# Sovik-Ghosh/SFM

Hardware: AMD Instinct MI355X
Metric: BA LM-iterations/sec + descriptor-pairs/sec, 200 cams / 100k pts, 1->8 MI355X (higher is better)
Workload: dtype f64; 1 GPU; BA: 200 cams / 100000 pts / 1000000 obs, cam block 10 (reference 10-parameter block + regulariser), aligned residual order, Huber, SciPy-TRF control flow, fixed schedule; parallelism=points sharded over 1 rank(s), cameras replicated, RCCL all-reduce of [S|r], comm=single rank, seed=1004

## Files before the change

include/sfm_amd.h:

```cpp
#ifndef SFM_AMD_H
#define SFM_AMD_H

#include <stdint.h>

#ifdef __cplusplus
extern "C" {
#endif

typedef struct sfm_ctx* sfm_handle;

enum { SFM_OK = 0, SFM_ERR_ARG = -1, SFM_ERR_HIP = -2, SFM_ERR_WORKSPACE = -3, SFM_ERR_NUMERIC = -4 };

int         sfm_create(int device, sfm_handle* out);
void        sfm_destroy(sfm_handle h);
const char* sfm_last_error(sfm_handle h);
int         sfm_set_stream(sfm_handle h, void* hip_stream);
int         sfm_synchronize(sfm_handle h);
const char* sfm_version(void);
int         sfm_copy_to_host(sfm_handle h, void* dst_host, const void* src_device, int64_t bytes);

int sfm_cgs_persist_enable(sfm_handle h, int enabled);
int sfm_cgs_persist_enabled(sfm_handle h);

enum { SFM_PROF_LIN_OBS = 0,
       SFM_PROF_LIN_REST = 1,
       SFM_PROF_BUILD_G = 2,
       SFM_PROF_SCHUR = 3,
       SFM_PROF_CHOL = 4,
       SFM_PROF_TRSV = 5,
       SFM_PROF_BACKSUB = 6,
       SFM_PROF_STEP = 7,
       SFM_PROF_KNN = 8,
       SFM_PROF_SCHUR_ITEMS = 9,
       SFM_PROF_FUND_HYP = 10,
       SFM_PROF_PNP_HYP = 11,
       SFM_PROF_POSE_VOTE = 12,
       SFM_PROF_FEAT_SCORE = 13,
       SFM_PROF_FEAT_SELECT = 14,
       SFM_PROF_FEAT_SCATTER = 15,
       SFM_PROF_FEAT_BLUR = 16,
       SFM_PROF_FEAT_DESCRIBE = 17,
       SFM_PROF_ESS_SOLVE = 18,
       SFM_PROF_ESS_SCORE = 19,
       SFM_PROF_HOM_HYP = 20,
       SFM_PROF_COUNT = 21 };
int sfm_set_profiling(sfm_handle h, int enabled);
int sfm_profile_read(sfm_handle h, int slot, double* total_ms_host, int64_t* count_host);

enum {
  SFM_METRIC_L2_U8   = 0,
  SFM_METRIC_L2_F32  = 1,
  SFM_METRIC_HAMMING = 2
};

int sfm_match_workspace_bytes(int metric, int64_t nq, int64_t nt, int dim, int64_t* bytes_host);

int sfm_match_knn2(sfm_handle h, int metric, const void* q, int64_t nq, const void* t, int64_t nt,
                   int dim, int32_t* idx1, int32_t* idx2, float* d1, float* d2,
                   void* workspace, int64_t workspace_bytes);

int sfm_match_ratio(sfm_handle h, int64_t nq, const int32_t* idx1, const float* d1, const float* d2,
                    double ratio, int32_t* query_idx, int32_t* train_idx, float* dist,
                    int64_t* n_matches, void* workspace, int64_t workspace_bytes);

int sfm_match_batched_workspace_bytes(int metric, int32_t n_seg, const int64_t* q_beg_host, const int64_t* q_end_host,
                                      const int64_t* t_beg_host, const int64_t* t_end_host, int64_t nq_rows,
                                      int64_t nt_rows, int64_t* n_out_host, int64_t* bytes_host);
int sfm_match_knn2_batched(sfm_handle h, int metric, const void* q, int64_t nq_rows, const void* t, int64_t nt_rows,
                           int dim, int32_t n_seg, const int64_t* q_beg_host, const int64_t* q_end_host,
                           const int64_t* t_beg_host, const int64_t* t_end_host, int32_t* idx1, int32_t* idx2,
                           float* d1, float* d2, int64_t* out_ptr_device, void* workspace, int64_t workspace_bytes);
int sfm_match_ratio_batched(sfm_handle h, int64_t n_out, int32_t n_seg, const int64_t* out_ptr_device, const int32_t* idx1,
                            const float* d1, const float* d2, double ratio, int32_t* query_idx, int32_t* train_idx,
                            float* dist, int64_t* seg_match_ptr_device, void* workspace, int64_t workspace_bytes);

int sfm_match_f32_to_u8(sfm_handle h, const float* src, int64_t n_elems, uint8_t* dst, int32_t* all_integral);

int sfm_guided_workspace_bytes(int metric, int32_t n_seg, const int64_t* q_beg_host, const int64_t* q_end_host,
                               const int64_t* t_beg_host, const int64_t* t_end_host, int64_t* n_out_host, int64_t* bytes_host);
int sfm_guided_match(sfm_handle h, int metric, const void* desc, int64_t n_rows, int dim, const float* xy, int32_t n_seg,
                     const int64_t* q_beg_host, const int64_t* q_end_host, const int64_t* t_beg_host, const int64_t* t_end_host,
                     const double* F, double gate_px, double ratio, double max_distance, int cross_check, int32_t* query_idx,
                     int32_t* train_idx, float* distance, int32_t* n_candidates, int64_t* seg_ptr, void* workspace,
                     int64_t workspace_bytes);


enum { SFM_CAMERA_SOLVER_AUTO = 0,
       SFM_CAMERA_SOLVER_CHOLESKY = 1,
       SFM_CAMERA_SOLVER_CG = 2 };
enum { SFM_BA_FP64 = 0,
       SFM_BA_MIXED = 1 };
enum { SFM_UV_AS_GIVEN = 0,
       SFM_UV_REFERENCE_PAIRING = 1 };
typedef struct {
  int32_t n_cams, n_pts, cam_dim, apply_reg;
  int64_t n_obs;
  const int32_t* cam_idx;
  const int32_t* pt_idx;
  const double*  uv;
  double fx0, fy0, cx0, cy0;
  double width, height, reg_weight;
  int32_t precision;
  int32_t camera_solver;
  int32_t uv_pairing;
  int32_t reserved;
} sfm_ba_desc;

typedef struct sfm_ba_prob* sfm_ba_problem;

typedef int (*sfm_reduce_fn)(void* user, void* data, int64_t count, int op);

enum { SFM_COMM_ID_BYTES = 128 };
int sfm_comm_unique_id(sfm_handle h, void* id_host);
int sfm_comm_init_rank(sfm_handle h, const void* id_host, int32_t n_ranks, int32_t rank);
int sfm_comm_adopt(sfm_handle h, void* nccl_comm, int32_t n_ranks, int32_t rank);
int sfm_comm_destroy(sfm_handle h);
int sfm_comm_info(sfm_handle h, int32_t* n_ranks_host, int32_t* rank_host);
int sfm_comm_allreduce(sfm_handle h, double* data, int64_t count, int op);
int sfm_comm_reduce_hook(void* handle_as_user, void* data, int64_t count, int op);

int  sfm_ba_create_problem(sfm_handle h, const sfm_ba_desc* desc, sfm_ba_problem* out);
void sfm_ba_destroy_problem(sfm_ba_problem p);

typedef struct {
  int64_t n_obs, n_pairs, n_items, n_cchunks, xcd_max_items;
  const int32_t* pt_ptr;
  const int32_t* cam_ptr;
  const int32_t* cam_obs;
  const int32_t* blk_ptr;
  const int32_t* pair_k;
  const int32_t* pair_k2;
  const int32_t* item_ptr;
  const int32_t* item_beg;
  const int32_t* item_end;
  const int32_t* xcd_ptr;
  const int32_t* xcd_items;
  const int32_t* cch_ptr;
  const int32_t* cch_beg;
  const int32_t* cch_end;
} sfm_ba_structure;
int sfm_ba_get_structure(sfm_ba_problem p, sfm_ba_structure* out_host);
int sfm_ba_get_item_descriptors(sfm_ba_problem p, const int32_t** first, const int32_t** stride, const int32_t** count);

typedef struct {
  int64_t total_bytes;
  int64_t rec_off, rec_stride;
  int64_t recB_off;
  int64_t B_off, gc_off;
  int64_t Cp_off, gp_off;
  int64_t reduce_lin_off, reduce_lin_count;
  int64_t gmax_off;
  int64_t reduce_S_off, reduce_S_count;
  int64_t reduce_Sp_off, reduce_Sp_count;
  int64_t reduce_q_off, reduce_q_count;
  int64_t reduce_step_off, reduce_step_count;
  int64_t pc_off, pp_off;
  int64_t scalars_off;
  int64_t G_off;
  int64_t cg_Ap_off, cg_M_off;
} sfm_ba_layout;

enum { SFM_SC_COST = 0, SFM_SC_GNORM2 = 1, SFM_SC_GINF = 2, SFM_SC_PNORM2 = 3, SFM_SC_PQ = 4,
       SFM_SC_JS2 = 5, SFM_SC_GTS = 6, SFM_SC_COST_NEW = 7, SFM_SC_SNORM2 = 8, SFM_SC_XNEW_NORM2 = 9,
       SFM_SC_CHOL_FAIL = 10 ,
       SFM_SC_HDIAG = 11 , SFM_SC_COUNT = 16 };

int sfm_ba_get_layout(sfm_ba_problem p, sfm_ba_layout* out_host);
int sfm_ba_bind_workspace(sfm_handle h, sfm_ba_problem p, void* workspace, int64_t workspace_bytes);

int sfm_ba_cost(sfm_handle h, sfm_ba_problem p, const double* x);
int sfm_ba_reproj_errors(sfm_handle h, sfm_ba_problem p, const double* x, int shared_k, double* err_out);

int sfm_ba_residual_norm2(sfm_handle h, sfm_ba_problem p, const double* x, int shared_k, double* out_host);

int sfm_reproj_errors(sfm_handle h, int32_t n_cams, int32_t cam_dim, int64_t n_obs, const int32_t* cam_idx,
                      const int32_t* pt_idx, const double* uv, const double* x, double fx, double fy, double cx,
                      double cy, int shared_k, double* err_out);

int sfm_ba_linearize(sfm_handle h, sfm_ba_problem p, const double* x);
int sfm_ba_finish_linearize(sfm_handle h, sfm_ba_problem p);

int sfm_ba_schur_build(sfm_handle h, sfm_ba_problem p, double alpha);
int sfm_ba_pack_system(sfm_handle h, sfm_ba_problem p);
int sfm_ba_unpack_system(sfm_handle h, sfm_ba_problem p);
int sfm_ba_schur_solve(sfm_handle h, sfm_ba_problem p, double alpha, int want_q);
int sfm_ba_finish_solve(sfm_handle h, sfm_ba_problem p, int want_q);

int sfm_ba_solve_pcg(sfm_handle h, sfm_ba_problem p, double alpha, int want_q, double rtol, int32_t max_iter,
                     sfm_reduce_fn reduce, void* reduce_user, int32_t* iters_host);

int sfm_ba_step(sfm_handle h, sfm_ba_problem p, const double* x, double scale, double* x_new);
int sfm_ba_finish_step(sfm_handle h, sfm_ba_problem p, const double* x, double scale, const double* x_new);

int sfm_ba_read_scalars(sfm_handle h, sfm_ba_problem p, double* out_host);
int sfm_ba_set_sharded(sfm_handle h, sfm_ba_problem p, int sharded);
int sfm_ba_solver_stats(sfm_ba_problem p, int64_t* cg_iters_host, int64_t* cg_fallbacks_host);

int sfm_ba_pcg_stats(sfm_ba_problem p, int64_t* fallbacks_host, double* worst_relres_host);

enum { SFM_SOLVER_DENSE = 0, SFM_SOLVER_PCG = 1 };
typedef struct {
  double ftol, xtol, gtol;
  int32_t max_nfev;
  int32_t max_outer;
  int32_t check_tolerances;
  int32_t solver;
  double  pcg_rtol;
  int32_t pcg_max_iter;
  int32_t reserved;
} sfm_trf_options;
typedef struct {
  double cost, optimality;
  int32_t nfev, njev, status;
  int32_t n_solves, n_outer;
  int32_t cg_iters;
} sfm_trf_result;
typedef struct sfm_trf_state_s* sfm_trf_state;
int  sfm_ba_trf_begin(sfm_handle h, sfm_ba_problem p, double* x, const sfm_trf_options* opt,
                      sfm_reduce_fn reduce, void* reduce_user, sfm_trf_state* out);
int  sfm_ba_trf_outer(sfm_trf_state st, int* more);
int  sfm_ba_trf_result(sfm_trf_state st, sfm_trf_result* out);
int  sfm_ba_trf_trace(sfm_trf_state st, double* out_host, int32_t capacity_trials);
void sfm_ba_trf_end(sfm_trf_state st);
int  sfm_ba_run_trf(sfm_handle h, sfm_ba_problem p, double* x, const sfm_trf_options* opt,
                    sfm_reduce_fn reduce, void* reduce_user, sfm_trf_result* out);

int sfm_dense_cholesky(sfm_handle h, double* a, int32_t n, int32_t* fail_flag);
int sfm_dense_trsv(sfm_handle h, const double* l, int32_t n, double* b, int transpose);


int sfm_assoc_workspace_bytes(int64_t n_rows, int64_t* bytes_host);
int sfm_assoc_radius(sfm_handle h, const double* track_xy, const int64_t* t_ptr, const double* corr_xy,
                     const int64_t* m_ptr, int32_t n_seg, int64_t n_rows, double radius,
                     int32_t* out_row, int32_t* out_col, int64_t capacity, int64_t* n_pairs,
                     void* workspace, int64_t workspace_bytes);

int sfm_triangulate2(sfm_handle h, const double* proj, int32_t n_cams, const int32_t* cam0, const int32_t* cam1,
                     const double* x0, const double* x1, int64_t n, double max_err,
                     double* X, int32_t* valid, double* err);

int sfm_epipolar_errors(sfm_handle h, const double* F, const int64_t* seg_ptr, int32_t n_seg,
                        const float* pts1, const float* pts2, int64_t n, float threshold,
                        float* err, uint8_t* mask);

int sfm_fund_workspace_bytes(int64_t n_points, int32_t n_seg, int32_t n_hyp, int64_t* bytes_host);
int sfm_fund_draw_samples(sfm_handle h, const int64_t* seg_ptr, int32_t n_seg, int32_t n_hyp, uint64_t seed,
                          int32_t* samples);
int sfm_fund_ransac(sfm_handle h, const int64_t* seg_ptr, int32_t n_seg, const float* pts1, const float* pts2,
                    int64_t n, const int32_t* samples, int32_t n_hyp, double threshold, int32_t refine,
                    double* F, uint8_t* mask, int32_t* n_inliers, int32_t* status, int32_t* hyp_count,
                    int32_t* refined, void* workspace, int64_t workspace_bytes);

int sfm_pnp_workspace_bytes(int64_t n_points, int32_t n_seg, int32_t n_hyp, int64_t* bytes_host);
int sfm_pnp_draw_samples(sfm_handle h, const int64_t* seg_ptr, int32_t n_seg, int32_t n_hyp, uint64_t seed,
                         int32_t* samples);
int sfm_pnp_ransac(sfm_handle h, const int64_t* seg_ptr, int32_t n_seg, const double* X, const float* uv, int64_t n,
                   const double* Kseg, const int32_t* samples, int32_t n_hyp, double threshold, int32_t refine,
                   double* Rt , uint8_t* mask, int32_t* n_inliers, int32_t* status,
                   int32_t* hyp_count , int32_t* refined , void* workspace,
                   int64_t workspace_bytes);

int sfm_ess_workspace_bytes(int64_t n_points, int32_t n_seg, int32_t n_hyp, int64_t* bytes_host);
int sfm_ess_draw_samples(sfm_handle h, const int64_t* seg_ptr, int32_t n_seg, int32_t n_hyp, uint64_t seed,
                         int32_t* samples);
int sfm_ess_ransac(sfm_handle h, const int64_t* seg_ptr, int32_t n_seg, const float* pts1, const float* pts2, int64_t n,
                   const double* Kseg , const int32_t* samples , int32_t n_hyp,
                   double threshold , int32_t refine, double* E , uint8_t* mask,
                   int32_t* n_inliers, int32_t* status, int32_t* hyp_count ,
                   int32_t* refined , void* workspace, int64_t workspace_bytes);

int sfm_hom_workspace_bytes(int64_t n_points, int32_t n_seg, int32_t n_hyp, int64_t* bytes_host);
int sfm_hom_draw_samples(sfm_handle h, const int64_t* seg_ptr, int32_t n_seg, int32_t n_hyp, uint64_t seed,
                         int32_t* samples);
int sfm_hom_ransac(sfm_handle h, const int64_t* seg_ptr, int32_t n_seg, const float* pts1, const float* pts2,
                   int64_t n, const int32_t* samples, int32_t n_hyp, double threshold, int32_t refine,
                   double* H, uint8_t* mask, int32_t* n_inliers, int32_t* status, int32_t* hyp_count,
                   int32_t* refined, void* workspace, int64_t workspace_bytes);

int sfm_pose_workspace_bytes(int64_t n_points, int32_t n_seg, int64_t* bytes_host);
int sfm_pose_recover(sfm_handle h, const int64_t* seg_ptr, int32_t n_seg, const float* pts1, const float* pts2,
                     int64_t n, const double* EorF , int32_t is_fundamental,
                     const double* Kseg , const uint8_t* mask_in , double dist,
                     double* R, double* t, int32_t* n_good, int32_t* status, uint8_t* mask_out,
                     double* X , int32_t* cand_count ,
                     double* cand_pose , int32_t* winner ,
                     void* workspace, int64_t workspace_bytes);

int sfm_tracks_workspace_bytes(int64_t n_nodes, int64_t n_edges, int64_t* bytes_host);
int sfm_tracks_build(sfm_handle h, const int64_t* kp_ptr, int32_t n_img, int64_t n_nodes, const int64_t* seg_ptr,
                     int32_t n_seg, const int32_t* pair_img , const int32_t* query_idx,
                     const int32_t* train_idx, const uint8_t* mask , int64_t n_edges, int32_t min_len,
                     int32_t policy, int64_t* track_ptr, int32_t* obs_image, int32_t* obs_kp, uint8_t* track_conflict,
                     int32_t* node_track, int64_t* counts, int64_t cap_tracks, int64_t cap_obs, void* workspace,
                     int64_t workspace_bytes);

enum { SFM_TRI_OK = 0,
       SFM_TRI_TOO_FEW_VIEWS = 1,
       SFM_TRI_DEGENERATE = 2,
       SFM_TRI_BEHIND = 3,
       SFM_TRI_LOW_ANGLE = 4,
       SFM_TRI_HIGH_ERROR = 5,
       SFM_TRI_STATUS_COUNT = 6 };
int sfm_triangulate_tracks_workspace_bytes(int32_t n_cams, int64_t* bytes_host);
int sfm_triangulate_tracks(sfm_handle h, const double* proj, int32_t n_cams, const int32_t* cam_of_image, int32_t n_img,
                           const int64_t* kp_ptr, const double* kp_xy, int64_t n_nodes, const int64_t* track_ptr,
                           int64_t n_tracks, const int32_t* obs_image, const int32_t* obs_kp, int64_t n_obs,
                           int32_t min_views, int32_t refine_iters, double max_error, double min_angle_deg, double* X,
                           int32_t* status, int32_t* n_views, double* max_err, int64_t* counts ,
                           void* workspace, int64_t workspace_bytes);

enum { SFM_EVAL_NO_POINT = -1 };
int sfm_tracks_evaluate(sfm_handle h, const double* proj, int32_t n_cams, const int32_t* cam_of_image, int32_t n_img,
                        const int64_t* kp_ptr, const double* kp_xy, int64_t n_nodes, const int64_t* track_ptr,
                        int64_t n_tracks, const int32_t* obs_image, const int32_t* obs_kp, int64_t n_obs,
                        const double* X, const uint8_t* has_point, int32_t min_views, double max_error,
                        double min_angle_deg, int32_t* status, int32_t* n_views, double* max_err,
                        double* obs_err , int64_t* counts ,
                        void* workspace, int64_t workspace_bytes);

enum { SFM_TRI_ROBUST_PAIRS = 64 };
int sfm_triangulate_tracks_robust_workspace_bytes(int32_t n_cams, int64_t n_tracks, int64_t* bytes_host);
int sfm_triangulate_tracks_robust(sfm_handle h, const double* proj, int32_t n_cams, const int32_t* cam_of_image,
                                  int32_t n_img, const int64_t* kp_ptr, const double* kp_xy, int64_t n_nodes,
                                  const int64_t* track_ptr, int64_t n_tracks, const int32_t* obs_image,
                                  const int32_t* obs_kp, int64_t n_obs, int32_t min_views, int32_t refine_iters,
                                  double max_error, double min_angle_deg, double* X, int32_t* status, int32_t* n_views,
                                  int32_t* n_inliers, double* max_err, uint8_t* obs_inlier ,
                                  int64_t* counts , void* workspace, int64_t workspace_bytes);
int sfm_tracks_classify(sfm_handle h, const double* proj, int32_t n_cams, const int32_t* cam_of_image, int32_t n_img,
                        const int64_t* kp_ptr, const double* kp_xy, int64_t n_nodes, const int64_t* track_ptr,
                        int64_t n_tracks, const int32_t* obs_image, const int32_t* obs_kp, int64_t n_obs,
                        const double* X, const uint8_t* has_point, int32_t min_views, double max_error,
                        double min_angle_deg, int32_t* status, int32_t* n_views, int32_t* n_inliers, double* max_err,
                        uint8_t* obs_inlier , double* obs_err ,
                        int64_t* counts , void* workspace, int64_t workspace_bytes);

int sfm_resection_workspace_bytes(int64_t n_nodes, int64_t* bytes_host);
int sfm_tracks_resection(sfm_handle h, const int64_t* kp_ptr, int32_t n_img, int64_t n_nodes, const double* kp_xy,
                         const int32_t* node_track, const int32_t* cam_of_image, const double* X ,
                         const uint8_t* has_point , int64_t n_tracks,
                         int64_t* seg_ptr , int32_t* corr_node, int32_t* corr_track,
                         double* corr_X , float* corr_uv , int64_t cap_corr,
                         int64_t* total, void* workspace, int64_t workspace_bytes);

int sfm_orb_default_pattern(int8_t base[256][4]);
int sfm_orb_rotate_pattern(const int8_t base[256][4], int8_t rot[30][256][4]);
int sfm_features_workspace_bytes(int32_t n_img, const int64_t* img_off_host, int64_t* bytes_host);
int sfm_features_detect(sfm_handle h, const uint8_t* images, const uint8_t* masks ,
                        const int64_t* img_off , const int32_t* heights ,
                        const int32_t* widths , int32_t n_img, int32_t threshold, int32_t edge,
                        int32_t max_features, int64_t* kp_ptr , void* workspace,
                        int64_t workspace_bytes);
int sfm_features_describe(sfm_handle h, const uint8_t* images, const int64_t* img_off ,
                          const int32_t* heights , const int32_t* widths , int32_t n_img,
                          const int64_t* kp_ptr , int64_t n_kp, const int8_t* rot_pattern ,
                          int32_t* xy , uint8_t* score, uint8_t* angle_bin,
                          uint8_t* desc , uint8_t* blurred_out , void* workspace,
                          int64_t workspace_bytes);

int sfm_features_pyramid_sizes(int32_t n_img, const int32_t* heights, const int32_t* widths, int32_t n_levels, int32_t num,
                               int32_t den, int64_t* lvl_off , int32_t* lvl_heights,
                               int32_t* lvl_widths);
int sfm_features_pyramid_workspace_bytes(int32_t n_img, int32_t n_levels, int64_t* bytes_host);
int sfm_features_pyramid(sfm_handle h, const uint8_t* images, const uint8_t* masks ,
                         const int64_t* img_off , const int32_t* heights ,
                         const int32_t* widths , int32_t n_img, int32_t n_levels, int32_t num, int32_t den,
                         uint8_t* lvl_images, uint8_t* lvl_masks , void* workspace,
                         int64_t workspace_bytes);
int sfm_features_merge_workspace_bytes(int32_t n_img, int32_t n_levels, int64_t* bytes_host);
int sfm_features_merge_count(sfm_handle h, const int64_t* lvl_kp_ptr ,
                             const uint8_t* lvl_score, int32_t n_img, int32_t n_levels, int32_t max_features,
                             int64_t* kp_ptr , void* workspace, int64_t workspace_bytes);
int sfm_features_merge_gather(sfm_handle h, const int64_t* lvl_kp_ptr, const int32_t* lvl_xy, const uint8_t* lvl_score,
                              const uint8_t* lvl_angle_bin, const uint8_t* lvl_desc, const int32_t* lvl_heights ,
                              const int32_t* lvl_widths , int32_t n_img, int32_t n_levels,
                              const int64_t* kp_ptr , int64_t n_kp, float* xy ,
                              uint8_t* level, uint8_t* score, uint8_t* angle_bin, uint8_t* desc ,
                              int32_t* src, void* workspace, int64_t workspace_bytes);

int sfm_depth_workspace_bytes(int32_t n_img, int32_t n_ref, int64_t n_entries, int64_t* bytes_host);
int sfm_depth_census(sfm_handle h, const uint8_t* images, const int64_t* img_off , const int32_t* heights ,
                     const int32_t* widths , int32_t n_img, uint64_t* census ,
                     void* workspace, int64_t workspace_bytes);
int sfm_depth_sweep(sfm_handle h, const uint64_t* census, const int64_t* img_off , const int32_t* heights ,
                    const int32_t* widths , int32_t n_img, int32_t n_ref, const int32_t* ref_image ,
                    const int64_t* src_ptr , const int32_t* src_image ,
                    const double* warps , const int64_t* plane_ptr ,
                    const double* plane_depth , int32_t radius, int32_t* plane, uint16_t* cost, float* depth,
                    void* workspace, int64_t workspace_bytes);
int sfm_depth_filter(sfm_handle h, const int64_t* img_off , const int32_t* heights ,
                     const int32_t* widths , int32_t n_img, int32_t n_ref, const int32_t* ref_image ,
                     const int64_t* src_ptr , const int32_t* src_image ,
                     const double* warps , const double* backproj ,
                     const float* depth, const uint16_t* cost, const int32_t* max_cost ,
                     double rel_tol, int32_t min_consistent, uint8_t* n_consistent, uint8_t* keep,
                     double* xyz , void* workspace, int64_t workspace_bytes);

int sfm_depth_fuse_workspace_bytes(int32_t n_img, int32_t n_ref, int64_t n_entries, int64_t n_out, int64_t* bytes_host);
int sfm_depth_fuse_mark(sfm_handle h, const int64_t* img_off , const int32_t* heights ,
                        const int32_t* widths , int32_t n_img, int32_t n_ref, const int32_t* ref_image ,
                        const int64_t* src_ptr , const int32_t* src_image ,
                        const double* warps , const double* backproj ,
                        const float* depth, const uint8_t* keep, const double* xyz, double rel_tol, int32_t normal_step,
                        double normal_jump, float* normal_map , uint8_t* agree_mask, uint8_t* owner,
                        int64_t* pt_ptr , void* workspace, int64_t workspace_bytes);
int sfm_depth_fuse_gather(sfm_handle h, const int64_t* img_off , const int32_t* heights ,
                          const int32_t* widths , int32_t n_img, int32_t n_ref, const int32_t* ref_image ,
                          const int64_t* src_ptr , const int32_t* src_image ,
                          const double* warps , const float* depth, const double* xyz,
                          const float* normal_map, const uint8_t* agree_mask, const uint8_t* owner,
                          const int64_t* pt_ptr , int64_t n_points, double* points ,
                          float* normals , uint8_t* n_views, int32_t* index ,
                          void* workspace, int64_t workspace_bytes);

int sfm_tsdf_workspace_bytes(int32_t n_ref, int64_t* bytes_host);
int sfm_tsdf_integrate(sfm_handle h, const int32_t* heights , const int32_t* widths , int32_t n_img,
                       int32_t n_ref, const int32_t* ref_image , const double* proj ,
                       const float* depth, const uint8_t* keep , const double* origin ,
                       double voxel, int32_t nx, int32_t ny, int32_t nz, double trunc, float* tsdf, uint16_t* weight,
                       void* workspace, int64_t workspace_bytes);
int sfm_mesh_workspace_bytes(int32_t nx, int32_t ny, int32_t nz, int64_t* bytes_host);
int sfm_mesh_mark(sfm_handle h, const float* tsdf, const uint16_t* weight, int32_t nx, int32_t ny, int32_t nz,
                  int32_t min_weight, int64_t* counts , void* workspace, int64_t workspace_bytes);
int sfm_mesh_emit(sfm_handle h, const float* tsdf, int32_t nx, int32_t ny, int32_t nz, const double* origin ,
                  double voxel, int64_t n_vertices, int64_t n_triangles, double* vertices, float* normals,
                  int32_t* triangles, void* workspace, int64_t workspace_bytes);

int sfm_mesh_colors_workspace_bytes(int32_t n_ref, int64_t* bytes_host);
int sfm_mesh_colors(sfm_handle h, const int32_t* heights , const int32_t* widths , int32_t n_img,
                    int32_t n_ref, const int32_t* ref_image , const double* proj ,
                    const double* centres , const float* depth, const uint8_t* keep ,
                    const uint8_t* pixels, int32_t channels, int64_t n_vertices, const double* vertices, const float* normals,
                    double tol, double min_cos, int32_t fill, uint8_t* colors, uint8_t* n_views, int32_t* best_view,
                    void* workspace, int64_t workspace_bytes);

int sfm_mesh_texture_size(int64_t n_triangles, int32_t texels, int32_t cells_per_row, int32_t* width_host, int32_t* height_host);
int sfm_mesh_texture_workspace_bytes(int32_t n_ref, int64_t* bytes_host);
int sfm_mesh_texture(sfm_handle h, const int32_t* heights , const int32_t* widths , int32_t n_img,
                     int32_t n_ref, const int32_t* ref_image , const double* proj ,
                     const double* centres , const float* depth, const uint8_t* keep ,
                     const uint8_t* pixels, int32_t channels, int64_t n_vertices, const double* vertices, const float* normals,
                     int64_t n_triangles, const int32_t* triangles, int32_t texels, int32_t cells_per_row, double tol,
                     double min_cos, int32_t fill, uint8_t* texture , uint8_t* views ,
                     float* uv , void* workspace, int64_t workspace_bytes);

#ifdef __cplusplus
}
#endif
#endif
```

sfm_amd/_lib.py:

```python
from __future__ import annotations

import ctypes as C
import os

_HERE = os.path.dirname(os.path.abspath(__file__))
LIB_PATH = os.environ.get("SFM_AMD_LIB") or os.path.join(_HERE, "lib", "libsfm_amd.so")

METRIC_L2_U8, METRIC_L2_F32, METRIC_HAMMING = 0, 1, 2
(SC_COST, SC_GNORM2, SC_GINF, SC_PNORM2, SC_PQ, SC_JS2, SC_GTS, SC_COST_NEW, SC_SNORM2,
 SC_XNEW_NORM2, SC_CHOL_FAIL, SC_HDIAG) = range(12)
SC_COUNT = 16
PROF_SLOTS = ("lin_obs", "lin_rest", "build_G", "schur", "chol", "trsv", "backsub", "step", "knn", "schur_items",
              "fund_hyp", "pnp_hyp", "pose_vote", "feat_score", "feat_select", "feat_scatter", "feat_blur", "feat_describe",
              "ess_solve", "ess_score", "hom_hyp")

i32, i64, f64, vp = C.c_int32, C.c_int64, C.c_double, C.c_void_p


PREC_FP64, PREC_MIXED = 0, 1
SOLVER_DENSE, SOLVER_PCG = 0, 1
CAMERA_AUTO, CAMERA_CHOLESKY, CAMERA_CG = 0, 1, 2
UV_AS_GIVEN, UV_REFERENCE_PAIRING = 0, 1
TRACKS_DROP, TRACKS_KEEP = 0, 1
(TRI_OK, TRI_TOO_FEW_VIEWS, TRI_DEGENERATE, TRI_BEHIND, TRI_LOW_ANGLE, TRI_HIGH_ERROR) = range(6)
EVAL_NO_POINT = -1


class BADesc(C.Structure):
    _fields_ = [("n_cams", i32), ("n_pts", i32), ("cam_dim", i32), ("apply_reg", i32),
                ("n_obs", i64),
                ("cam_idx", vp), ("pt_idx", vp), ("uv", vp),
                ("fx0", f64), ("fy0", f64), ("cx0", f64), ("cy0", f64),
                ("width", f64), ("height", f64), ("reg_weight", f64),
                ("precision", i32), ("camera_solver", i32), ("uv_pairing", i32), ("reserved", i32)]


class BAStructureView(C.Structure):
    _fields_ = ([(n, i64) for n in ("n_obs", "n_pairs", "n_items", "n_cchunks", "xcd_max_items")] +
                [(n, vp) for n in ("pt_ptr", "cam_ptr", "cam_obs", "blk_ptr", "pair_k", "pair_k2", "item_ptr",
                                   "item_beg", "item_end", "xcd_ptr", "xcd_items", "cch_ptr", "cch_beg", "cch_end")])


class TRFOptions(C.Structure):
    _fields_ = [("ftol", f64), ("xtol", f64), ("gtol", f64), ("max_nfev", i32), ("max_outer", i32),
                ("check_tolerances", i32), ("solver", i32), ("pcg_rtol", f64), ("pcg_max_iter", i32), ("reserved", i32)]


class TRFResultC(C.Structure):
    _fields_ = [("cost", f64), ("optimality", f64), ("nfev", i32), ("njev", i32), ("status", i32),
                ("n_solves", i32), ("n_outer", i32), ("cg_iters", i32)]


REDUCE_FN = C.CFUNCTYPE(C.c_int, vp, vp, i64, C.c_int)


class BALayout(C.Structure):
    _fields_ = [(n, i64) for n in (
        "total_bytes", "rec_off", "rec_stride", "recB_off", "B_off", "gc_off", "Cp_off", "gp_off",
        "reduce_lin_off", "reduce_lin_count", "gmax_off", "reduce_S_off", "reduce_S_count", "reduce_Sp_off", "reduce_Sp_count",
        "reduce_q_off", "reduce_q_count", "reduce_step_off", "reduce_step_count",
        "pc_off", "pp_off", "scalars_off", "G_off", "cg_Ap_off", "cg_M_off")]


TRACK_SOURCE = (vp, i32, vp, i32, vp, vp, i64, vp, i64, vp, vp, i64)

SIGNATURES = {
    "sfm_create": (C.c_int, [C.c_int, C.POINTER(vp)]),
    "sfm_destroy": (None, [vp]),
    "sfm_last_error": (C.c_char_p, [vp]),
    "sfm_set_stream": (C.c_int, [vp, vp]),
    "sfm_synchronize": (C.c_int, [vp]),
    "sfm_version": (C.c_char_p, []),
    "sfm_cgs_persist_enable": (C.c_int, [vp, C.c_int]),
    "sfm_cgs_persist_enabled": (C.c_int, [vp]),
    "sfm_set_profiling": (C.c_int, [vp, C.c_int]),
    "sfm_profile_read": (C.c_int, [vp, C.c_int, C.POINTER(f64), C.POINTER(i64)]),
    "sfm_match_workspace_bytes": (C.c_int, [C.c_int, i64, i64, C.c_int, C.POINTER(i64)]),
    "sfm_match_knn2": (C.c_int, [vp, C.c_int, vp, i64, vp, i64, C.c_int, vp, vp, vp, vp, vp, i64]),
    "sfm_match_ratio": (C.c_int, [vp, i64, vp, vp, vp, f64, vp, vp, vp, vp, vp, i64]),
    "sfm_match_f32_to_u8": (C.c_int, [vp, vp, i64, vp, vp]),
    "sfm_match_batched_workspace_bytes": (C.c_int, [C.c_int, i32, vp, vp, vp, vp, i64, i64, C.POINTER(i64), C.POINTER(i64)]),
    "sfm_match_knn2_batched": (C.c_int, [vp, C.c_int, vp, i64, vp, i64, C.c_int, i32, vp, vp, vp, vp, vp, vp, vp, vp, vp, vp, i64]),
    "sfm_match_ratio_batched": (C.c_int, [vp, i64, i32, vp, vp, vp, vp, f64, vp, vp, vp, vp, vp, i64]),
    "sfm_guided_workspace_bytes": (C.c_int, [C.c_int, i32, vp, vp, vp, vp, C.POINTER(i64), C.POINTER(i64)]),
    "sfm_guided_match": (C.c_int, [vp, C.c_int, vp, i64, C.c_int, vp, i32, vp, vp, vp, vp, vp, f64, f64, f64, C.c_int,
                                   vp, vp, vp, vp, vp, vp, i64]),
    "sfm_copy_to_host": (C.c_int, [vp, vp, vp, i64]),
    "sfm_comm_unique_id": (C.c_int, [vp, vp]),
    "sfm_comm_init_rank": (C.c_int, [vp, vp, i32, i32]),
    "sfm_comm_adopt": (C.c_int, [vp, vp, i32, i32]),
    "sfm_comm_destroy": (C.c_int, [vp]),
    "sfm_comm_info": (C.c_int, [vp, C.POINTER(i32), C.POINTER(i32)]),
    "sfm_comm_allreduce": (C.c_int, [vp, vp, i64, C.c_int]),
    "sfm_comm_reduce_hook": (C.c_int, [vp, vp, i64, C.c_int]),
    "sfm_ba_create_problem": (C.c_int, [vp, C.POINTER(BADesc), C.POINTER(vp)]),
    "sfm_ba_destroy_problem": (None, [vp]),
    "sfm_ba_get_structure": (C.c_int, [vp, C.POINTER(BAStructureView)]),
    "sfm_ba_get_item_descriptors": (C.c_int, [vp, C.POINTER(vp), C.POINTER(vp), C.POINTER(vp)]),
    "sfm_ba_get_layout": (C.c_int, [vp, C.POINTER(BALayout)]),
    "sfm_ba_set_sharded": (C.c_int, [vp, vp, C.c_int]),
    "sfm_ba_solver_stats": (C.c_int, [vp, C.POINTER(i64), C.POINTER(i64)]),
    "sfm_ba_pcg_stats": (C.c_int, [vp, C.POINTER(i64), C.POINTER(f64)]),
    "sfm_ba_bind_workspace": (C.c_int, [vp, vp, vp, i64]),
    "sfm_reproj_errors": (C.c_int, [vp, i32, i32, i64, vp, vp, vp, vp, f64, f64, f64, f64, C.c_int, vp]),
    "sfm_ba_solve_pcg": (C.c_int, [vp, vp, f64, C.c_int, f64, i32, REDUCE_FN, vp, C.POINTER(i32)]),
    "sfm_ba_trf_begin": (C.c_int, [vp, vp, vp, C.POINTER(TRFOptions), REDUCE_FN, vp, C.POINTER(vp)]),
    "sfm_ba_trf_outer": (C.c_int, [vp, C.POINTER(C.c_int)]),
    "sfm_ba_trf_result": (C.c_int, [vp, C.POINTER(TRFResultC)]),
    "sfm_ba_trf_trace": (C.c_int, [vp, vp, i32]),
    "sfm_ba_trf_end": (None, [vp]),
    "sfm_ba_run_trf": (C.c_int, [vp, vp, vp, C.POINTER(TRFOptions), REDUCE_FN, vp, C.POINTER(TRFResultC)]),
    "sfm_ba_cost": (C.c_int, [vp, vp, vp]),
    "sfm_ba_reproj_errors": (C.c_int, [vp, vp, vp, C.c_int, vp]),
    "sfm_ba_residual_norm2": (C.c_int, [vp, vp, vp, C.c_int, C.POINTER(f64)]),
    "sfm_ba_linearize": (C.c_int, [vp, vp, vp]),
    "sfm_ba_finish_linearize": (C.c_int, [vp, vp]),
    "sfm_ba_schur_build": (C.c_int, [vp, vp, f64]),
    "sfm_ba_pack_system": (C.c_int, [vp, vp]),
    "sfm_ba_unpack_system": (C.c_int, [vp, vp]),
    "sfm_ba_schur_solve": (C.c_int, [vp, vp, f64, C.c_int]),
    "sfm_ba_finish_solve": (C.c_int, [vp, vp, C.c_int]),
    "sfm_ba_step": (C.c_int, [vp, vp, vp, f64, vp]),
    "sfm_ba_finish_step": (C.c_int, [vp, vp, vp, f64, vp]),
    "sfm_ba_read_scalars": (C.c_int, [vp, vp, C.POINTER(f64)]),
    "sfm_dense_cholesky": (C.c_int, [vp, vp, i32, vp]),
    "sfm_dense_trsv": (C.c_int, [vp, vp, i32, vp, C.c_int]),
    "sfm_assoc_workspace_bytes": (C.c_int, [i64, C.POINTER(i64)]),
    "sfm_assoc_radius": (C.c_int, [vp, vp, vp, vp, vp, i32, i64, f64, vp, vp, i64, vp, vp, i64]),
    "sfm_triangulate2": (C.c_int, [vp, vp, i32, vp, vp, vp, vp, i64, f64, vp, vp, vp]),
    "sfm_epipolar_errors": (C.c_int, [vp, vp, vp, i32, vp, vp, i64, C.c_float, vp, vp]),
    "sfm_fund_workspace_bytes": (C.c_int, [i64, i32, i32, C.POINTER(i64)]),
    "sfm_fund_draw_samples": (C.c_int, [vp, vp, i32, i32, C.c_uint64, vp]),
    "sfm_fund_ransac": (C.c_int, [vp, vp, i32, vp, vp, i64, vp, i32, f64, i32, vp, vp, vp, vp, vp, vp, vp, i64]),
    "sfm_pnp_workspace_bytes": (C.c_int, [i64, i32, i32, C.POINTER(i64)]),
    "sfm_pnp_draw_samples": (C.c_int, [vp, vp, i32, i32, C.c_uint64, vp]),
    "sfm_pnp_ransac": (C.c_int, [vp, vp, i32, vp, vp, i64, vp, vp, i32, f64, i32, vp, vp, vp, vp, vp, vp, vp, i64]),
    "sfm_ess_workspace_bytes": (C.c_int, [i64, i32, i32, C.POINTER(i64)]),
    "sfm_ess_draw_samples": (C.c_int, [vp, vp, i32, i32, C.c_uint64, vp]),
    "sfm_ess_ransac": (C.c_int, [vp, vp, i32, vp, vp, i64, vp, vp, i32, f64, i32, vp, vp, vp, vp, vp, vp, vp, i64]),
    "sfm_hom_workspace_bytes": (C.c_int, [i64, i32, i32, C.POINTER(i64)]),
    "sfm_hom_draw_samples": (C.c_int, [vp, vp, i32, i32, C.c_uint64, vp]),
    "sfm_hom_ransac": (C.c_int, [vp, vp, i32, vp, vp, i64, vp, i32, f64, i32, vp, vp, vp, vp, vp, vp, vp, i64]),
    "sfm_pose_workspace_bytes": (C.c_int, [i64, i32, C.POINTER(i64)]),
    "sfm_pose_recover": (C.c_int, [vp, vp, i32, vp, vp, i64, vp, i32, vp, vp, f64, vp, vp, vp, vp, vp, vp, vp, vp, vp, vp, i64]),
    "sfm_tracks_workspace_bytes": (C.c_int, [i64, i64, C.POINTER(i64)]),
    "sfm_tracks_build": (C.c_int, [vp, vp, i32, i64, vp, i32, vp, vp, vp, vp, i64, i32, i32, vp, vp, vp, vp, vp, vp, i64, i64, vp, i64]),
    "sfm_triangulate_tracks_workspace_bytes": (C.c_int, [i32, C.POINTER(i64)]),
    "sfm_triangulate_tracks": (C.c_int, [vp, *TRACK_SOURCE, i32, i32, f64, f64, vp, vp, vp, vp, vp, vp, i64]),
    "sfm_tracks_evaluate": (C.c_int, [vp, *TRACK_SOURCE, vp, vp, i32, f64, f64, vp, vp, vp, vp, vp, vp, i64]),
    "sfm_triangulate_tracks_robust_workspace_bytes": (C.c_int, [i32, i64, C.POINTER(i64)]),
    "sfm_triangulate_tracks_robust": (C.c_int, [vp, *TRACK_SOURCE, i32, i32, f64, f64, vp, vp, vp, vp, vp, vp, vp, vp, i64]),
    "sfm_tracks_classify": (C.c_int, [vp, *TRACK_SOURCE, vp, vp, i32, f64, f64, vp, vp, vp, vp, vp, vp, vp, vp, i64]),
    "sfm_resection_workspace_bytes": (C.c_int, [i64, C.POINTER(i64)]),
    "sfm_tracks_resection": (C.c_int, [vp, vp, i32, i64, vp, vp, vp, vp, vp, i64, vp, vp, vp, vp, vp, i64, vp, vp, i64]),
    "sfm_orb_default_pattern": (C.c_int, [vp]),
    "sfm_orb_rotate_pattern": (C.c_int, [vp, vp]),
    "sfm_features_workspace_bytes": (C.c_int, [i32, vp, C.POINTER(i64)]),
    "sfm_features_detect": (C.c_int, [vp, vp, vp, vp, vp, vp, i32, i32, i32, i32, vp, vp, i64]),
    "sfm_features_describe": (C.c_int, [vp, vp, vp, vp, vp, i32, vp, i64, vp, vp, vp, vp, vp, vp, vp, i64]),
    "sfm_features_pyramid_sizes": (C.c_int, [i32, vp, vp, i32, i32, i32, vp, vp, vp]),
    "sfm_features_pyramid_workspace_bytes": (C.c_int, [i32, i32, C.POINTER(i64)]),
    "sfm_features_pyramid": (C.c_int, [vp, vp, vp, vp, vp, vp, i32, i32, i32, i32, vp, vp, vp, i64]),
    "sfm_features_merge_workspace_bytes": (C.c_int, [i32, i32, C.POINTER(i64)]),
    "sfm_features_merge_count": (C.c_int, [vp, vp, vp, i32, i32, i32, vp, vp, i64]),
    "sfm_features_merge_gather": (C.c_int, [vp, vp, vp, vp, vp, vp, vp, vp, i32, i32, vp, i64, vp, vp, vp, vp, vp, vp, vp, i64]),
    "sfm_depth_workspace_bytes":(C.c_int, [i32, i32, i64, C.POINTER(i64)]),
    "sfm_depth_census": (C.c_int, [vp, vp, vp, vp, vp, i32, vp, vp, i64]),
    "sfm_depth_sweep": (C.c_int, [vp, vp, vp, vp, vp, i32, i32, vp, vp, vp, vp, vp, vp, i32, vp, vp, vp, vp, i64]),
    "sfm_depth_filter": (C.c_int, [vp, vp, vp, vp, i32, i32, vp, vp, vp, vp, vp, vp, vp, vp, f64, i32, vp, vp, vp, vp, i64]),
    "sfm_depth_fuse_workspace_bytes": (C.c_int, [i32, i32, i64, i64, C.POINTER(i64)]),
    "sfm_depth_fuse_mark": (C.c_int, [vp, vp, vp, vp, i32, i32, vp, vp, vp, vp, vp, vp, vp, vp, f64, i32, f64, vp, vp, vp, vp, vp, i64]),
    "sfm_depth_fuse_gather": (C.c_int, [vp, vp, vp, vp, i32, i32, vp, vp, vp, vp, vp, vp, vp, vp, vp, vp, i64, vp, vp, vp, vp, vp, i64]),
    "sfm_tsdf_workspace_bytes": (C.c_int, [i32, C.POINTER(i64)]),
    "sfm_tsdf_integrate": (C.c_int, [vp, vp, vp, i32, i32, vp, vp, vp, vp, vp, f64, i32, i32, i32, f64, vp, vp, vp, i64]),
    "sfm_mesh_workspace_bytes": (C.c_int, [i32, i32, i32, C.POINTER(i64)]),
    "sfm_mesh_mark": (C.c_int, [vp, vp, vp, i32, i32, i32, i32, vp, vp, i64]),
    "sfm_mesh_emit": (C.c_int, [vp, vp, i32, i32, i32, vp, f64, i64, i64, vp, vp, vp, vp, i64]),
    "sfm_mesh_colors_workspace_bytes": (C.c_int, [i32, C.POINTER(i64)]),
    "sfm_mesh_colors": (C.c_int, [vp, vp, vp, i32, i32, vp, vp, vp, vp, vp, vp, i32, i64, vp, vp, f64, f64, i32, vp, vp, vp, vp, i64]),
    "sfm_mesh_texture_size": (C.c_int, [i64, i32, i32, C.POINTER(i32), C.POINTER(i32)]),
    "sfm_mesh_texture_workspace_bytes": (C.c_int, [i32, C.POINTER(i64)]),
    "sfm_mesh_texture": (C.c_int, [vp, vp, vp, i32, i32, vp, vp, vp, vp, vp, vp, i32, i64, vp, vp, i64, vp, i32, i32, f64, f64, i32, vp, vp, vp,
                                   vp, i64]),
}

_lib = None


class SfmError(RuntimeError):
    pass


class SfmNumericError(SfmError):
    """SFM_ERR_NUMERIC: a damped system was not positive definite, a solve stalled or a step was not finite."""


def load():
    global _lib
    if _lib is None:
        if not os.path.exists(LIB_PATH):
            raise SfmError(f"{LIB_PATH} not built: run `python -m sfm_amd.build` "
                           "(hipcc --offload-arch=gfx950); there is no CPU fallback")
        try:
            import torch
        except ImportError:
            pass
        lib = C.CDLL(LIB_PATH)
        for name, (res, args) in SIGNATURES.items():
            fn = getattr(lib, name)
            fn.restype = res
            fn.argtypes = args
        _lib = lib
    return _lib


class Handle:

    def __init__(self, device=0):
        import torch
        if not torch.cuda.is_available():
            raise SfmError("sfm_amd needs a ROCm GPU (gfx950); none is visible and there is no CPU fallback")
        self.lib = load()
        self.device = int(device)
        self._h = vp()
        rc = self.lib.sfm_create(self.device, C.byref(self._h))
        if rc != 0:
            raise SfmError(f"sfm_create(device={device}) failed with {rc}")
        self.bind_stream()

    def bind_stream(self):
        import torch
        s = torch.cuda.current_stream(self.device).cuda_stream
        self.check(self.lib.sfm_set_stream(self._h, vp(s)), "sfm_set_stream")

    def check(self, rc, what):
        if rc != 0:
            msg = self.lib.sfm_last_error(self._h)
            raise (SfmNumericError if rc == -4 else SfmError)(f"{what} failed ({rc}): {msg.decode() if msg else ''}")

    def call(self, name, *args):
        self.check(getattr(self.lib, name)(self._h, *args), name)

    def set_profiling(self, on):
        self.call("sfm_set_profiling", 1 if on else 0)

    def profile(self):
        out = {}
        for i, name in enumerate(PROF_SLOTS):
            ms, cnt = f64(), i64()
            self.call("sfm_profile_read", i, C.byref(ms), C.byref(cnt))
            out[name] = (ms.value, cnt.value)
        return out

    def __del__(self):
        try:
            if self._h:
                self.lib.sfm_destroy(self._h)
                self._h = vp()
        except Exception:
            pass


_handles = {}


def _release_handles():
    import gc
    gc.collect()
    _handles.clear()


import atexit
atexit.register(_release_handles)


def get_handle(device=0):
    h = _handles.get(device)
    if h is None:
        h = _handles[device] = Handle(device)
    else:
        h.bind_stream()
    return h
```

sfm_amd/csrc/ba.hip:

```cpp
#include "ba_internal.h"
#include "ba_device.h"
#include <atomic>

static int64_t g_stride(int64_t D) { return D == 10 ? 32 : 3 * D; }
Lay ba_layout(int64_t C, int64_t P, int64_t N, int64_t D, int64_t n_items, int64_t n_cchunks, int precision) {
  Lay L;
  int64_t o = 0, n = C * D;
  auto take = [&](int64_t cnt) { int64_t r = o; o = align_up(o + cnt, 32); return r; };
  const int64_t es = precision == SFM_BA_MIXED ? 4 : 8;
  auto take_rec = [&](int64_t elems) { return take((elems * es + 7) / 8); };
  L.nblk_obs = (N + 255) / 256;
  L.nblk_pt = (P + 255) / 256;
  L.recA = take_rec(N * 2 * D);
  L.recB = take_rec(N * 8);
  L.campre = take(C * CAMPRE);
  L.campre2 = take(C * CAMPRE);
  L.B = take(C * D * D);
  L.gc = take(n);
  L.Cp = take(P * 6);
  L.gp = take(P * 3);
  L.Linv = take(P * 6);
  L.e = take(P * 3);
  L.v = take(P * 3);
  L.tmp3 = take(N * 3);
  L.G = take(N * g_stride(D));
  L.eobs = take(N * 3);
  L.red_lin = take(2 * n + 2);
  L.gmax = take(2);
  L.red_S = take(n * n + n);
  L.red_q = take(n + 2);
  L.red_step = take(8);
  L.pc = take(n);
  L.pp = take(P * 3);
  L.y = take(n);
  L.tvec = take(n);
  L.scalars = take(SFM_SC_COUNT);
  L.part_obs = take(L.nblk_obs * 2 * 4 + 4);
  L.part_pt = take(L.nblk_pt * 4);
  L.part_x = take(((n + 3 * P + 255) / 256) * 2 + 2);
  L.cost_reg = take(C * 4);
  L.regrec = take(C * 20);
  L.dense = take(dense_ws_doubles((int)n));
  L.sch_part = take(n_items * D * D);
  L.cch_part = take(n_cchunks * 16);
  L.cbl_part = take(n_cchunks * (D * D + D));
  L.cg_r = take(n); L.cg_z = take(n); L.cg_p = take(n); L.cg_Ap = take(n);
  L.cg_M = take(C * D * D); L.cg_Minv = take(C * D * D);
  L.cg_scal = take(CG_SCAL_WORDS);
  L.cg_mail = take(4 * n);
  L.total = o;
  return L;
}

extern "C" int sfm_ba_get_layout(sfm_ba_problem p, sfm_ba_layout* out) {
  if (!p || !out) return SFM_ERR_ARG;
  const Lay& L = p->L;
  const int64_t n = (int64_t)p->n_cams * p->cam_dim;
  const int64_t es = p->precision == SFM_BA_MIXED ? 4 : 8;
  out->total_bytes = L.total * 8;
  out->rec_off = L.recA * 8; out->rec_stride = 2 * p->cam_dim * es;
  out->recB_off = L.recB * 8;
  out->B_off = L.B * 8; out->gc_off = L.gc * 8;
  out->Cp_off = L.Cp * 8; out->gp_off = L.gp * 8;
  out->reduce_lin_off = L.red_lin * 8; out->reduce_lin_count = 2 * n + 2;
  out->gmax_off = L.gmax * 8;
  out->reduce_S_off = L.red_S * 8; out->reduce_S_count = n * n + n;
  out->reduce_Sp_off = (L.dense + dense_ws_lm_offset((int)n)) * 8;
  out->reduce_Sp_count = n * (n + 1) / 2 + n;
  out->reduce_q_off = L.red_q * 8; out->reduce_q_count = n + 2;
  out->reduce_step_off = L.red_step * 8; out->reduce_step_count = 5;
  out->pc_off = L.pc * 8; out->pp_off = L.pp * 8;
  out->scalars_off = L.scalars * 8;
  out->G_off = L.G * 8;
  out->cg_Ap_off = L.cg_Ap * 8; out->cg_M_off = L.cg_M * 8;
  return SFM_OK;
}

__device__ __forceinline__ void point_factor_vals(const double* __restrict__ c, const double* __restrict__ g, double alpha,
                                                  double (&m)[6], double (&ev)[3]) {
  const double a00 = c[0] + alpha, a10 = c[1], a20 = c[2], a11 = c[3] + alpha, a21 = c[4], a22 = c[5] + alpha;
  const double l00 = sqrt(a00), l10 = a10 / l00, l20 = a20 / l00;
  const double l11 = sqrt(a11 - l10 * l10), l21 = (a21 - l20 * l10) / l11;
  const double l22 = sqrt(a22 - l20 * l20 - l21 * l21);
  const double m00 = 1.0 / l00, m11 = 1.0 / l11, m22 = 1.0 / l22;
  const double m10 = -l10 * m00 * m11, m21 = -l21 * m11 * m22;
  const double m20 = -(l20 * m00 + l21 * m10) * m22;
  m[0] = m00; m[1] = m10; m[2] = m11; m[3] = m20; m[4] = m21; m[5] = m22;
  const double g0 = g[0], g1 = g[1], g2 = g[2];
  ev[0] = m00 * g0;
  ev[1] = m10 * g0 + m11 * g1;
  ev[2] = m20 * g0 + m21 * g1 + m22 * g2;
}

template <int D, typename T, typename TG, int GS>
__global__ __launch_bounds__(256) void k_build_G(int64_t N, const int* __restrict__ pt_idx,
                                                 const T* __restrict__ recA, const T* __restrict__ recB,
                                                 double* __restrict__ Linv, TG* __restrict__ G,
                                                 double* __restrict__ e, double* __restrict__ eobs,
                                                 const double* __restrict__ Cp, const double* __restrict__ gp, double alpha, int P,
                                                 unsigned nblk_obs, double* __restrict__ cg_scal ) {
  static_assert(GS % 2 == 0 && GS >= 3 * D, "G blocks are written as 16-byte pieces");
  if (cg_scal && blockIdx.x == 0 && threadIdx.x < CG_SCAL_WORDS) cg_scal[threadIdx.x] = 0.0;
  if (blockIdx.x >= nblk_obs) {
    const int j = (int)(blockIdx.x - nblk_obs) * 256 + (int)threadIdx.x;
    if (j < P) {
      double m[6], ev[3];
      point_factor_vals(Cp + (size_t)j * 6, gp + (size_t)j * 3, alpha, m, ev);
#pragma unroll
      for (int q = 0; q < 6; ++q) Linv[(size_t)j * 6 + q] = m[q];
#pragma unroll
      for (int q = 0; q < 3; ++q) e[(size_t)j * 3 + q] = ev[q];
    }
    return;
  }
  constexpr int WA = 2 * D, LDA = WA + 1, LDB = 9, LDG = GS + 1;
  constexpr int VE = 16 / (int)sizeof(T);
  constexpr int NA = WA / VE, NB = 8 / VE;
  static_assert(WA % VE == 0 && 8 % VE == 0, "record rows are whole 16-byte pieces");
  constexpr int IN_DOUBLES = 256 * (LDA + LDB), OUT_DOUBLES = 256 * LDG;
  __shared__ double s_buf[IN_DOUBLES > OUT_DOUBLES ? IN_DOUBLES : OUT_DOUBLES];
  double* s_jp = s_buf + 256 * LDA;
  typedef T vec_t __attribute__((ext_vector_type(VE)));
  const int tid = threadIdx.x;
  const int64_t k0 = (int64_t)blockIdx.x * 256;
  const int nvalid = (int)((N - k0) < 256 ? (N - k0) : 256);
  const bool live = tid < nvalid;
  const int64_t k = k0 + tid;
  const int64_t pj = live ? pt_idx[k] : 0;
  vec_t la[NA], lb[NB];
  {
    const vec_t* inA = (const vec_t*)(recA + (size_t)k0 * WA);
    const vec_t* inB = (const vec_t*)(recB + (size_t)k0 * 8);
#pragma unroll
    for (int j = 0; j < NA; ++j) { const int i = tid + 256 * j; la[j] = i * VE < nvalid * WA ? inA[i] : (vec_t)(T)0; }
#pragma unroll
    for (int j = 0; j < NB; ++j) { const int i = tid + 256 * j; lb[j] = i * VE < nvalid * 8 ? inB[i] : (vec_t)(T)0; }
  }
  double cpj[6], gpj[3];
#pragma unroll
  for (int q = 0; q < 6; ++q) cpj[q] = Cp[(size_t)pj * 6 + q];
#pragma unroll
  for (int q = 0; q < 3; ++q) gpj[q] = gp[(size_t)pj * 3 + q];
#pragma unroll
  for (int j = 0; j < NA; ++j)
#pragma unroll
    for (int v = 0; v < VE; ++v) { const int i = (tid + 256 * j) * VE + v, t = i / WA, q = i - t * WA; s_buf[t * LDA + q] = (double)la[j][v]; }
#pragma unroll
  for (int j = 0; j < NB; ++j)
#pragma unroll
    for (int v = 0; v < VE; ++v) { const int i = (tid + 256 * j) * VE + v; s_jp[(i >> 3) * LDB + (i & 7)] = (double)lb[j][v]; }
  __syncthreads();
  double mq[6], eq[3];
  point_factor_vals(cpj, gpj, alpha, mq, eq);
  const double m00 = mq[0], m10 = mq[1], m11 = mq[2], m20 = mq[3], m21 = mq[4], m22 = mq[5];
  const double e0 = eq[0], e1 = eq[1], e2 = eq[2];
  double g[3 * D];
  {
    const double* jp = &s_jp[tid * LDB];
    const double j0 = jp[0], j1 = jp[1], j2 = jp[2], j3 = jp[3], j4 = jp[4], j5 = jp[5];
    const double v00 = j0 * m00, v01 = j0 * m10 + j1 * m11, v02 = j0 * m20 + j1 * m21 + j2 * m22;
    const double v10 = j3 * m00, v11 = j3 * m10 + j4 * m11, v12 = j3 * m20 + j4 * m21 + j5 * m22;
    const double* my = &s_buf[tid * LDA];
#pragma unroll
    for (int a = 0; a < D; ++a) {
      const double c0 = my[a], c1 = my[D + a];
      g[a] = c0 * v00 + c1 * v10;
      g[D + a] = c0 * v01 + c1 * v11;
      g[2 * D + a] = c0 * v02 + c1 * v12;
    }
  }
  if (live) { eobs[k * 3] = e0; eobs[k * 3 + 1] = e1; eobs[k * 3 + 2] = e2; }
  __syncthreads();
  {
    double* my = &s_buf[tid * LDG];
#pragma unroll
    for (int q = 0; q < 3 * D; ++q) my[q] = g[q];
#pragma unroll
    for (int q = 3 * D; q < GS; ++q) my[q] = 0.0;
  }
  __syncthreads();
  {
    typedef TG pair_t __attribute__((ext_vector_type(2)));
    pair_t* outp = (pair_t*)(G + (size_t)k0 * GS);
    constexpr int HP = GS / 2;
#pragma unroll
    for (int j = 0; j < HP; ++j) {
      const int i = tid + 256 * j;
      if (i < nvalid * HP) {
        const int t = i / HP, q = 2 * (i - t * HP);
        pair_t v; v.x = (TG)s_buf[t * LDG + q]; v.y = (TG)s_buf[t * LDG + q + 1];
        outp[i] = v;
      }
    }
  }
}

#ifndef SFM_SCHUR_WAVES_D10
#define SFM_SCHUR_WAVES_D10 5
#endif
#ifndef SFM_SCHUR_U_D10
#define SFM_SCHUR_U_D10 8
#endif
#ifndef SFM_SCHUR_WAVES_D6
#define SFM_SCHUR_WAVES_D6 8
#endif
#ifndef SFM_SCHUR_U_D6
#define SFM_SCHUR_U_D6 4
#endif
#ifdef SFM_SCHUR_WAVES
#undef SFM_SCHUR_WAVES_D10
#undef SFM_SCHUR_WAVES_D6
#define SFM_SCHUR_WAVES_D10 SFM_SCHUR_WAVES
#define SFM_SCHUR_WAVES_D6 SFM_SCHUR_WAVES
#endif
#ifdef SFM_SCHUR_U
#undef SFM_SCHUR_U_D10
#undef SFM_SCHUR_U_D6
#define SFM_SCHUR_U_D10 SFM_SCHUR_U
#define SFM_SCHUR_U_D6 SFM_SCHUR_U
#endif
#ifndef SFM_SCHUR_STAMPS
#define SFM_SCHUR_STAMPS 0
#endif
#if SFM_SCHUR_STAMPS
constexpr int SCHUR_STAMP_WAVES = 1 << 16;
__device__ unsigned long long g_schur_stamps[SCHUR_STAMP_WAVES * 4];
extern "C" int sfm_debug_schur_stamps(unsigned long long* dst, int n_words) {
  return (int)hipMemcpyFromSymbol(dst, HIP_SYMBOL(g_schur_stamps), (size_t)n_words * 8, 0, hipMemcpyDeviceToHost);
}
#define SCHUR_STAMP_BEGIN() const unsigned long long stamp_t0 = __builtin_amdgcn_s_memrealtime()
#define SCHUR_STAMP_END(npairs, isdiag) do { const unsigned wv = blockIdx.x * SFM_SCHUR_WG_WAVES + (threadIdx.x >> 6); if ((threadIdx.x & 63) == 0 && wv < SCHUR_STAMP_WAVES) { \
    unsigned long long* o = g_schur_stamps + (size_t)wv * 4; \
    o[0] = stamp_t0; o[1] = __builtin_amdgcn_s_memrealtime(); \
    o[2] = ((unsigned long long)(unsigned)(npairs) << 32) | (unsigned)__builtin_amdgcn_s_getreg((31 << 11) | 4); \
    o[3] = (unsigned)__builtin_amdgcn_s_getreg((31 << 11) | 20) | ((unsigned long long)((isdiag) ? 1 : 0) << 32); } } while (0)
#else
#define SCHUR_STAMP_BEGIN() do {} while (0)
#define SCHUR_STAMP_END(npairs, isdiag) do {} while (0)
#endif
#ifndef SFM_SCHUR_WG_WAVES
#define SFM_SCHUR_WG_WAVES 1
#endif
template <int D, typename T, int GS>
__global__ __launch_bounds__(64 * SFM_SCHUR_WG_WAVES) __attribute__((amdgpu_waves_per_eu(D == 6 ? SFM_SCHUR_WAVES_D6 : SFM_SCHUR_WAVES_D10, D == 6 ? SFM_SCHUR_WAVES_D6 : SFM_SCHUR_WAVES_D10))) void k_schur_items(const int* __restrict__ xcd_ptr, const int* __restrict__ xcd_items,
                                                     const int* __restrict__ it_first,
                                                     const int* __restrict__ it_stride,
                                                     const int* __restrict__ it_cnt,
                                                     const int* __restrict__ pair_k, const int* __restrict__ pair_k2,
                                                     const T* __restrict__ G, double* __restrict__ part,
                                                     const int* __restrict__ cam_idx,
                                                     const int* __restrict__ item_ptr, const int* __restrict__ cch_ptr, int n_cams,
                                                     const double* __restrict__ eobs, double* __restrict__ cch_part,
                                                     int fuse_rhs) {
  typedef int chunk_t __attribute__((ext_vector_type(4)));
  constexpr int BB = GS * (int)sizeof(T);
  static_assert(BB % 16 == 0, "a G block must be a whole number of 16-byte chunks");
  static_assert(D < 16, "column D of the 16 x 16 product is the right-hand side");
  constexpr int CH = BB / 16;
  constexpr int BPL = 64 / CH;
  constexpr int UMAX = D == 6 ? SFM_SCHUR_U_D6 : SFM_SCHUR_U_D10;
  constexpr int U = (64 + BPL - 1) / BPL < UMAX ? (64 + BPL - 1) / BPL : UMAX;
  constexpr int PB = U * BPL;
  constexpr int WGW = SFM_SCHUR_WG_WAVES;
  __shared__ __attribute__((aligned(16))) char s_stage[WGW][2][BPL * BB + 16];
  __shared__ double s_e[WGW][64][3];
  const int lane = threadIdx.x & 63, w = threadIdx.x >> 6;
  const int grp = blockIdx.x & 7;
  const int pos = xcd_ptr[grp] + (blockIdx.x >> 3) * WGW + w;
  if (pos >= xcd_ptr[grp + 1]) return;
  SCHUR_STAMP_BEGIN();
  const int it = __builtin_amdgcn_readfirstlane(xcd_items[pos]);
  const int first = __builtin_amdgcn_readfirstlane(it_first[it]), stride = __builtin_amdgcn_readfirstlane(it_stride[it]);
  const int n = __builtin_amdgcn_readfirstlane(it_cnt[it]);
  const int row = lane & 15, m = lane >> 4;
  const int lb = lane / CH, lc = lane - lb * CH;
  const bool loader = lb < BPL;
  char* sA = s_stage[w][0];
  char* sB = s_stage[w][1];
  const char* Gb = (const char*)G;
  v4d acc = {0.0, 0.0, 0.0, 0.0};
  const int k_first = __builtin_amdgcn_readfirstlane(pair_k[first]), k2_first = __builtin_amdgcn_readfirstlane(pair_k2[first]);
  const bool diag = fuse_rhs && k_first == k2_first;
  constexpr int NM = (3 * BPL + 3) / 4;
  const bool krow = row < D, ke_lane = row == D;
  constexpr int ZSLOT = BPL * GS;
  int koff[NM];
#pragma unroll
  for (int j = 0; j < NM; ++j) {
    const int sl = 4 * j + m, pi = (sl * 11) >> 5;
    koff[j] = (pi < BPL && krow) ? pi * GS + (sl - 3 * pi) * D + row : ZSLOT;
  }
  if (lane < 2) { ((double*)sA)[ZSLOT + lane] = 0.0; ((double*)sB)[ZSLOT + lane] = 0.0; }
  auto run = [&](auto diag_c) __attribute__((always_inline)) {
    constexpr bool DIAG = decltype(diag_c)::value;
    int kk_n = lane < n ? pair_k[first + lane * stride] : 0;
    int kk2_n = DIAG ? kk_n : (lane < n ? pair_k2[first + lane * stride] : 0);
    for (int base = 0; base < n; base += 64) {
      const int kk = kk_n, kk2 = kk2_n;
      if (base + 64 < n) {
        const int jn = base + 64 + lane;
        kk_n = jn < n ? pair_k[first + jn * stride] : 0;
        kk2_n = DIAG ? kk_n : (jn < n ? pair_k2[first + jn * stride] : 0);
      }
      const int cnt = (n - base) < 64 ? (n - base) : 64;
      if (DIAG) {
        const double* ej = eobs + (size_t)kk * 3;
        const double e0 = ej[0], e1 = ej[1], e2 = ej[2];
        s_e[w][lane][0] = e0; s_e[w][lane][1] = e1; s_e[w][lane][2] = e2;
      }
      for (int u0 = 0; u0 < cnt; u0 += PB) {
        chunk_t ra[U], rb[U];
        if (u0 + PB <= cnt) {
#pragma unroll
          for (int t = 0; t < U; ++t) {
            const int p = u0 + t * BPL + (loader ? lb : BPL - 1);
            ra[t] = *(const chunk_t*)(Gb + (size_t)(unsigned)__shfl(kk, p, 64) * BB + 16 * lc);
            if (!DIAG) rb[t] = *(const chunk_t*)(Gb + (size_t)(unsigned)__shfl(kk2, p, 64) * BB + 16 * lc);
          }
        } else
#pragma unroll
        for (int t = 0; t < U; ++t) {
          const int p = u0 + t * BPL + lb;
          const int k = __shfl(kk, p & 63, 64);
          const bool ok = loader && p < cnt;
          ra[t] = ok ? *(const chunk_t*)(Gb + (size_t)k * BB + 16 * lc) : (chunk_t){0, 0, 0, 0};
          if (!DIAG) {
            const int k2 = __shfl(kk2, p & 63, 64);
            rb[t] = ok ? *(const chunk_t*)(Gb + (size_t)k2 * BB + 16 * lc) : (chunk_t){0, 0, 0, 0};
          }
        }
#pragma unroll
        for (int t = 0; t < U; ++t) {
          if (u0 + t * BPL >= cnt) break;
          if (loader) {
            *(chunk_t*)(sA + lb * BB + 16 * lc) = ra[t];
            if (!DIAG) *(chunk_t*)(sB + lb * BB + 16 * lc) = rb[t];
          }
          __builtin_amdgcn_fence(__ATOMIC_RELEASE, "wavefront");
          __builtin_amdgcn_fence(__ATOMIC_ACQUIRE, "wavefront");
          const int nb = (cnt - (u0 + t * BPL)) < BPL ? (cnt - (u0 + t * BPL)) : BPL;
          const int nm = (3 * nb + 3) >> 2;
          constexpr int PFN = D == 6 ? 1 : NM;
#pragma unroll
          for (int j0 = 0; j0 < NM; j0 += PFN) {
            if (j0 >= nm) break;
            double av[PFN], bv[PFN];
#pragma unroll
            for (int q = 0; q < PFN; ++q) {
              const int j = j0 + q;
              if (j < NM) {
                const int ko = koff[j];
                av[q] = (double)((const T*)sA)[ko];
                if (DIAG) {
                  const int sl = 4 * j + m, pi = (sl * 11) >> 5;
                  bv[q] = ko != ZSLOT ? av[q] : ((ke_lane && pi < nb) ? s_e[w][u0 + t * BPL + pi][sl - 3 * pi] : 0.0);
                } else bv[q] = (double)((const T*)sB)[ko];
              }
            }
#pragma unroll
            for (int q = 0; q < PFN; ++q) {
              if (j0 + q >= nm || j0 + q >= NM) break;
              acc = __builtin_amdgcn_mfma_f64_16x16x4f64(av[q], bv[q], acc, 0, 0, 0);
            }
          }
          __builtin_amdgcn_fence(__ATOMIC_RELEASE, "wavefront");
        }
      }
    }
  };
  if (diag) run(std::true_type{}); else run(std::false_type{});
  const int col = lane & 15;
  if (col < D) {
#pragma unroll
    for (int i = 0; i < 4; ++i) {
      const int rr = (lane >> 4) + 4 * i;
      if (rr < D) part[(size_t)it * (D * D) + rr * D + col] = acc[i];
    }
  } else if (diag && col == D) {
    const int c = cam_idx[k_first];
    const int64_t blk = (int64_t)c * n_cams - (int64_t)c * (c - 1) / 2;
    const int ch = cch_ptr[c] + (it - item_ptr[blk]);
#pragma unroll
    for (int i = 0; i < 4; ++i) {
      const int rr = (lane >> 4) + 4 * i;
      if (rr < D) cch_part[(size_t)ch * 16 + rr] = acc[i];
    }
  }
  SCHUR_STAMP_END(n, diag);
}

template <int D>
__device__ __forceinline__ void diag_block_factor_lanes(const double* blk, int ld, double alpha, int i, int r,
                                                        double* __restrict__ Einv, double* __restrict__ Efac, double* __restrict__ cg_scal) {
  double Lr[D], Xc[D];
#pragma unroll
  for (int k = 0; k < D; ++k) Lr[k] = (k <= i) ? blk[i * ld + k] + (i == k ? alpha : 0.0) : 0.0;
  bool ok = true;
#pragma unroll
  for (int j = 0; j < D; ++j) {
    double sum = Lr[j];
#pragma unroll
    for (int k = 0; k < j; ++k) sum = fma(-Lr[k], Lr[k], sum);
    double piv = __shfl(sum, j, 64);
    if (!(piv > 0.0)) { ok = false; piv = 1.0; }
    const double l = sqrt(piv);
    double t = Lr[j];
#pragma unroll
    for (int k = 0; k < j; ++k) t = fma(-Lr[k], __shfl(Lr[k], j, 64), t);
    Lr[j] = (i == j) ? l : (i > j ? t / l : Lr[j]);
  }
#pragma unroll
  for (int rw = 0; rw < D; ++rw) {
    double sum = (rw == i) ? 1.0 : 0.0;
#pragma unroll
    for (int k = 0; k < rw; ++k) {
      const double lrk = __shfl(Lr[k], rw, 64);
      sum = (k >= i) ? fma(-lrk, Xc[k], sum) : sum;
    }
    const double lrr = __shfl(Lr[rw], rw, 64);
    Xc[rw] = (rw >= i) ? sum / lrr : 0.0;
  }
#pragma unroll
  for (int k = 0; k < D; ++k) {
    Efac[(size_t)r * D * D + i * D + k] = k <= i ? Lr[k] : 0.0;
    Einv[(size_t)r * D * D + k * D + i] = Xc[k];
  }
  if (!ok) cg_scal[CGS_FAIL] = 1.0;
}
template <int D, int ASM_NB>
__device__ __forceinline__ void strip_item_sums(int C, int r, int c_0, int nv, int e, const int* __restrict__ item_ptr,
                                                const double* __restrict__ part, const double* __restrict__ B, double (&v)[ASM_NB]) {
  const int rr = e / D, col = e - rr * D;
  const int eT = col * D + rr;
  int ib[ASM_NB], ie[ASM_NB], mx = 0;
#pragma unroll
  for (int j = 0; j < ASM_NB; ++j) {
    ib[j] = ie[j] = 0;
    if (j < nv) {
      const int c = c_0 + j;
      const int64_t blk = (int64_t)c * C - (int64_t)c * (c - 1) / 2 + (r - c);
      ib[j] = item_ptr[blk]; ie[j] = item_ptr[blk + 1];
    }
  }
#pragma unroll
  for (int j = 0; j < ASM_NB; ++j) { v[j] = 0.0; mx = (ie[j] - ib[j]) > mx ? (ie[j] - ib[j]) : mx; }
  for (int i = 0; i < mx; ++i) {
#pragma unroll
    for (int j = 0; j < ASM_NB; ++j)
      if (ib[j] + i < ie[j]) v[j] += part[(size_t)(ib[j] + i) * (D * D) + ((c_0 + j == r) ? e : eT)];
  }
#pragma unroll
  for (int j = 0; j < ASM_NB; ++j) {
    v[j] = -v[j];
    if (j < nv && c_0 + j == r) v[j] += B[(size_t)r * D * D + e];
  }
}
template <int D, int ASM_NB, bool ROUNDS>
__global__ __launch_bounds__(128) void k_schur_assemble(int C, const int* __restrict__ item_ptr,
                                                        const double* __restrict__ part,
                                                        const double* __restrict__ B, double* __restrict__ S, double* __restrict__ cg_scal,
                                                        const int* __restrict__ cch_ptr, const double* __restrict__ cch_part,
                                                        const double* __restrict__ gc, double* __restrict__ rhs_out,
                                                        double alpha, double* __restrict__ Einv , double* __restrict__ Efac) {
  if (blockIdx.y == 0 && threadIdx.x < 64) {
    const int cc = blockIdx.x, lane = threadIdx.x, sl = lane >> 4, a = lane & 15;
    double t = 0.0;
    for (int ch = cch_ptr[cc] + sl; ch < cch_ptr[cc + 1]; ch += 4) t += cch_part[(size_t)ch * 16 + a];
    const double t1 = __shfl(t, a + 16, 64), t2 = __shfl(t, a + 32, 64), t3 = __shfl(t, a + 48, 64);
    if (sl == 0 && a < D) rhs_out[cc * D + a] = gc[cc * D + a] - ((t + t1) + (t2 + t3));
  }
  __shared__ double sOut[D][ASM_NB * D + 1];
  const int r = blockIdx.x, c_0 = blockIdx.y * ASM_NB;
  if (c_0 > r) return;
  const int nv = (r - c_0 + 1) < ASM_NB ? (r - c_0 + 1) : ASM_NB;
  const int e = threadIdx.x;
  if (e < D * D) {
    const int rr = e / D, col = e - rr * D;
    if (ROUNDS) {
      double v[ASM_NB];
      strip_item_sums<D, ASM_NB>(C, r, c_0, nv, e, item_ptr, part, B, v);
#pragma unroll
      for (int j = 0; j < ASM_NB; ++j)
        if (j < nv) sOut[rr][j * D + col] = v[j];
    } else {
      const int eT = col * D + rr;
#pragma unroll
      for (int j = 0; j < ASM_NB; ++j)
        if (j < nv) {
          const int c = c_0 + j;
          const int64_t blk = (int64_t)c * C - (int64_t)c * (c - 1) / 2 + (r - c);
          const int src = (c == r) ? e : eT;
          double s = 0.0;
          for (int it = item_ptr[blk]; it < item_ptr[blk + 1]; ++it) s += part[(size_t)it * (D * D) + src];
          double v = -s;
          if (c == r) v += B[(size_t)c * D * D + e];
          sOut[rr][j * D + col] = v;
        }
    }
  }
  __syncthreads();
  if (Einv && r < c_0 + ASM_NB && e < D)
    diag_block_factor_lanes<D>(&sOut[0][(r - c_0) * D], ASM_NB * D + 1, alpha, e, r, Einv, Efac, cg_scal);
  const int n = C * D, W = nv * D;
  constexpr int WMAX = ASM_NB * D, NST = (D * WMAX + 127) / 128;
#pragma unroll
  for (int t = 0; t < NST; ++t) {
    const int idx = e + 128 * t;
    const int rr = idx / WMAX, col = idx - rr * WMAX;
    if (rr < D && col < W) S[(size_t)(r * D + rr) * n + c_0 * D + col] = sOut[rr][col];
  }
}

template <int D>
__global__ __launch_bounds__(128) void k_schur_diag(int C, const int* __restrict__ item_ptr, const double* __restrict__ part,
                                                    const double* __restrict__ B, double alpha, double* __restrict__ Einv,
                                                    double* __restrict__ Efac, double* __restrict__ cg_scal) {
  __shared__ double sBlk[D][D + 1];
  const int r = blockIdx.x, e = threadIdx.x;
  if (e < D * D) {
    const int rr = e / D, col = e - rr * D;
    const int64_t blk = (int64_t)r * C - (int64_t)r * (r - 1) / 2;
    double s = 0.0;
#pragma unroll 4
    for (int it = item_ptr[blk]; it < item_ptr[blk + 1]; ++it) s += part[(size_t)it * (D * D) + e];
    double v = -s;
    v += B[(size_t)r * D * D + e];
    sBlk[rr][col] = v;
  }
  __syncthreads();
  if (e < D) diag_block_factor_lanes<D>(&sBlk[0][0], D + 1, alpha, e, r, Einv, Efac, cg_scal);
}
template <int D, int ASM_NB>
__global__ __launch_bounds__(128) void k_schur_assemble_scaled(int C, const int* __restrict__ item_ptr, const double* __restrict__ part,
                                                               const double* __restrict__ B, double* __restrict__ St,
                                                               const int* __restrict__ cch_ptr, const double* __restrict__ cch_part,
                                                               const double* __restrict__ gc, double* __restrict__ rhs_out,
                                                               double* __restrict__ rhs_t, double alpha, const double* __restrict__ Einv) {
  constexpr int SCALED_BAND = 128 / D + 2;
  if (blockIdx.y == 0 && threadIdx.x < 64) {
    const int cc = blockIdx.x, lane = threadIdx.x, sl = lane >> 4, a = lane & 15;
    double t = 0.0;
    for (int ch = cch_ptr[cc] + sl; ch < cch_ptr[cc + 1]; ch += 4) t += cch_part[(size_t)ch * 16 + a];
    const double t1 = __shfl(t, a + 16, 64), t2 = __shfl(t, a + 32, 64), t3 = __shfl(t, a + 48, 64);
    const double rv = (sl == 0 && a < D) ? gc[cc * D + a] - ((t + t1) + (t2 + t3)) : 0.0;
    double ts = 0.0;
#pragma unroll
    for (int k = 0; k < D; ++k) ts += Einv[(size_t)cc * D * D + (a < D ? a : 0) * D + k] * __shfl(rv, k, 64);
    if (sl == 0 && a < D) { rhs_out[cc * D + a] = rv; rhs_t[cc * D + a] = ts; }
  }
  __shared__ double sOut[D][ASM_NB * D + 1];
  __shared__ double sE1[D * D], sE2[ASM_NB][D * D];
  const int r = blockIdx.x, c_0 = blockIdx.y * ASM_NB;
  if (c_0 > r) return;
  const int nv = (r - c_0 + 1) < ASM_NB ? (r - c_0 + 1) : ASM_NB;
  const int e = threadIdx.x;
  const int a = e / D, b = e - a * D;
  if (e < D * D) {
    double ev[ASM_NB + 1];
    ev[ASM_NB] = Einv[(size_t)r * D * D + e];
#pragma unroll
    for (int j = 0; j < ASM_NB; ++j) ev[j] = j < nv ? Einv[(size_t)(c_0 + j) * D * D + e] : 0.0;
    double v[ASM_NB];
    strip_item_sums<D, ASM_NB>(C, r, c_0, nv, e, item_ptr, part, B, v);
    sE1[e] = ev[ASM_NB];
#pragma unroll
    for (int j = 0; j < ASM_NB; ++j)
      if (j < nv) { sOut[a][j * D + b] = v[j]; sE2[j][e] = ev[j]; }
  }
  __syncthreads();
  const bool has_diag = r < c_0 + ASM_NB;
  const int jd = (r - c_0) * D;
  double dv = 0.0;
  if (has_diag && e < D * D) dv = (b <= a ? sOut[a][jd + b] : sOut[b][jd + a]) + (a == b ? alpha : 0.0);
  __syncthreads();
  if (has_diag && e < D * D) sOut[a][jd + b] = dv;
  __syncthreads();
  constexpr int RPT = 1;
  constexpr int RH = D / RPT;
  const int oj = e / RH, oh = e - oj * RH;
  const bool owner = e < ASM_NB * RH && oj < nv;
  double out[RPT][D];
  if (owner) {
#pragma unroll
    for (int q = 0; q < RPT; ++q) {
      const int ra = oh + q * RH;
      double tr[D];
#pragma unroll
      for (int bb = 0; bb < D; ++bb) tr[bb] = 0.0;
#pragma unroll
      for (int k = 0; k < D; ++k) {
        const double e1 = sE1[ra * D + k];
#pragma unroll
        for (int bb = 0; bb < D; ++bb) tr[bb] = fma(e1, sOut[k][oj * D + bb], tr[bb]);
        __builtin_amdgcn_sched_barrier(0);
      }
#pragma unroll
      for (int bb = 0; bb < D; ++bb) {
        double t = 0.0;
#pragma unroll
        for (int k = 0; k < D; ++k) t = fma(tr[k], sE2[oj][bb * D + k], t);
        out[q][bb] = t;
        __builtin_amdgcn_sched_barrier(0);
      }
    }
  }
  __syncthreads();
  if (owner) {
#pragma unroll
    for (int q = 0; q < RPT; ++q)
#pragma unroll
      for (int bb = 0; bb < D; ++bb) sOut[oh + q * RH][oj * D + bb] = out[q][bb];
  }
  __syncthreads();
  const int n = C * D, W = nv * D;
  constexpr int WMAX = ASM_NB * D, NST = (D * WMAX + 127) / 128;
#pragma unroll
  for (int t = 0; t < NST; ++t) {
    const int idx = e + 128 * t;
    const int rr = idx / WMAX, col = idx - rr * WMAX;
    if (rr < D && col < W) St[(size_t)(r * D + rr) * n + c_0 * D + col] = sOut[rr][col];
  }
  if (e < D * D) {
#pragma unroll
    for (int j = 0; j < ASM_NB; ++j) {
      const int c = c_0 + j;
      if (j < nv && c < r && r - c <= SCALED_BAND)
        St[(size_t)(c * D + a) * n + r * D + b] = sOut[b][j * D + a];
    }
  }
}

template <int D, typename T, int GS>
__global__ __launch_bounds__(256) void k_cam_reduce_chunks(const int* __restrict__ cch_beg, const int* __restrict__ cch_end,
                                                           const int* __restrict__ cam_obs, const int* __restrict__ cam_pt,
                                                           const T* __restrict__ G, const double* __restrict__ vec,
                                                           double* __restrict__ part) {
  static_assert(D % 2 == 0 && GS % 2 == 0 && GS <= 32, "16-byte pieces of a block: one per lane of a 16-lane group");
  typedef T pair_t __attribute__((ext_vector_type(2)));
  __shared__ double s[4][4][32];
  const int ch = blockIdx.x, tid = threadIdx.x, lane = tid & 63, w = tid >> 6;
  const int grp = lane >> 4, l16 = lane & 15;
  const int e0 = 2 * l16;
  const bool live = e0 < 3 * D;
  const int m = live ? e0 / D : 0;
  double acc0 = 0.0, acc1 = 0.0;
  const int beg = cch_beg[ch], end = cch_end[ch];
  constexpr int UNR = 4;
  for (int i0 = beg + w * 4 + grp; i0 < end; i0 += 16 * UNR) {
    int k[UNR], pj[UNR];
    pair_t g[UNR];
    double vm[UNR];
#pragma unroll
    for (int u = 0; u < UNR; ++u) { const int i = i0 + 16 * u; k[u] = i < end ? cam_obs[i] : -1; pj[u] = i < end ? cam_pt[i] : 0; }
#pragma unroll
    for (int u = 0; u < UNR; ++u) {
      g[u] = (k[u] >= 0 && live) ? *(const pair_t*)(G + (size_t)k[u] * GS + e0) : (pair_t){(T)0, (T)0};
    }
#pragma unroll
    for (int u = 0; u < UNR; ++u) vm[u] = k[u] >= 0 ? vec[(size_t)pj[u] * 3 + m] : 0.0;
#pragma unroll
    for (int u = 0; u < UNR; ++u)
      if (k[u] >= 0 && live) { acc0 += (double)g[u].x * vm[u]; acc1 += (double)g[u].y * vm[u]; }
  }
  s[w][grp][e0] = acc0; s[w][grp][e0 + 1] = acc1;
  __syncthreads();
  if (tid < 16) {
    double t = 0.0;
    if (tid < D) {
#pragma unroll
      for (int mm = 0; mm < 3; ++mm)
#pragma unroll
        for (int ww = 0; ww < 4; ++ww)
#pragma unroll
          for (int gg = 0; gg < 4; ++gg) t += s[ww][gg][mm * D + tid];
    }
    part[(size_t)ch * 16 + tid] = t;
  }
}
template <int D>
__global__ __launch_bounds__(256) void k_cam_reduce_final(int C, const int* __restrict__ cch_ptr, const double* __restrict__ part,
                                                          const double* __restrict__ base, double* __restrict__ out,
                                                          const double* __restrict__ sum_part = nullptr, int sum_nblk = 0, int sum_cnt = 0,
                                                          double* __restrict__ sum_dst = nullptr) {
  if (sum_part && blockIdx.x == gridDim.x - 1) {
    __shared__ double s_red[4];
    for (int q = 0; q < sum_cnt; ++q) {
      double t = 0.0;
      for (int i = threadIdx.x; i < sum_nblk; i += 256) t += sum_part[(size_t)i * sum_cnt + q];
      const double tt = block_sum256(t, s_red);
      if (threadIdx.x == 0) sum_dst[q] = tt;
    }
    return;
  }
  const int c = blockIdx.x * 4 + (threadIdx.x >> 6);
  if (c >= C) return;
  const int lane = threadIdx.x & 63, s = lane >> 4, a = lane & 15;
  double t = 0.0;
  for (int ch = cch_ptr[c] + s; ch < cch_ptr[c + 1]; ch += 4) t += part[(size_t)ch * 16 + a];
  const double t1 = __shfl(t, a + 16, 64), t2 = __shfl(t, a + 32, 64), t3 = __shfl(t, a + 48, 64);
  if (s == 0 && a < D) out[c * D + a] = (base ? base[c * D + a] : 0.0) - ((t + t1) + (t2 + t3));
}

constexpr int GTP_OBS = 64;
template <int D, typename T, int GS>
__global__ __launch_bounds__(256) void k_obs_Gtp(int64_t N, const int* __restrict__ cam_idx,
                                                 const T* __restrict__ G,
                                                 const double* __restrict__ pc, double* __restrict__ tmp3) {
  static_assert(D % 2 == 0 && GS % 2 == 0 && GS <= 32, "16-byte pieces of a block: one per lane of a 16-lane group");
  typedef T pair_t __attribute__((ext_vector_type(2)));
  __shared__ double s[GTP_OBS][17];
  const int tid = threadIdx.x, slot = tid >> 4, l16 = tid & 15;
  const int64_t k0 = (int64_t)blockIdx.x * GTP_OBS;
  const int e0 = 2 * l16;
  const int a = e0 % D;
  const bool live = e0 < 3 * D;
  pair_t g[GTP_OBS / 16];
  int cam[GTP_OBS / 16];
#pragma unroll
  for (int it = 0; it < GTP_OBS / 16; ++it) {
    const int64_t k = k0 + it * 16 + slot;
    const bool ok = live && k < N;
    g[it] = ok ? *(const pair_t*)(G + (size_t)k * GS + e0) : (pair_t)(T)0;
    cam[it] = ok ? cam_idx[k] : 0;
  }
#pragma unroll
  for (int it = 0; it < GTP_OBS / 16; ++it) {
    const double2 p = *(const double2*)(pc + (size_t)cam[it] * D + a);
    s[it * 16 + slot][l16] = (double)g[it].x * p.x + (double)g[it].y * p.y;
  }
  __syncthreads();
  if (tid < 3 * GTP_OBS) {
    const int sl = tid / 3, mm = tid - 3 * sl;
    const int64_t kk = k0 + sl;
    if (kk < N) {
      double u = 0.0;
#pragma unroll
      for (int j = 0; j < D / 2; ++j) u += s[sl][mm * (D / 2) + j];
      tmp3[kk * 3 + mm] = u;
    }
  }
}

__global__ __launch_bounds__(256) void k_backsub(int P, const int* __restrict__ pt_ptr,
                                                 const double* __restrict__ tmp3,
                                                 const double* __restrict__ Linv,
                                                 const double* __restrict__ e, double* __restrict__ pp,
                                                 double* __restrict__ v, double* __restrict__ part) {
  __shared__ double s_red[4];
  const int j = blockIdx.x * 256 + threadIdx.x;
  double p2 = 0.0, v2 = 0.0;
  if (j < P) {
    double u0 = e[(size_t)j * 3], u1 = e[(size_t)j * 3 + 1], u2 = e[(size_t)j * 3 + 2];
#pragma unroll 5
    for (int k = pt_ptr[j]; k < pt_ptr[j + 1]; ++k) {
      u0 += tmp3[(size_t)k * 3]; u1 += tmp3[(size_t)k * 3 + 1]; u2 += tmp3[(size_t)k * 3 + 2];
    }
    const double* M = Linv + (size_t)j * 6;
    const double q0 = -(M[0] * u0 + M[1] * u1 + M[3] * u2);
    const double q1 = -(M[2] * u1 + M[4] * u2);
    const double q2 = -(M[5] * u2);
    pp[(size_t)j * 3] = q0; pp[(size_t)j * 3 + 1] = q1; pp[(size_t)j * 3 + 2] = q2;
    const double w0 = M[0] * q0, w1 = M[1] * q0 + M[2] * q1, w2 = M[3] * q0 + M[4] * q1 + M[5] * q2;
    v[(size_t)j * 3] = w0; v[(size_t)j * 3 + 1] = w1; v[(size_t)j * 3 + 2] = w2;
    p2 = q0 * q0 + q1 * q1 + q2 * q2;
    v2 = w0 * w0 + w1 * w1 + w2 * w2;
  }
  double a = block_sum256(p2, s_red);
  double b = block_sum256(v2, s_red);
  if (threadIdx.x == 0) { part[blockIdx.x * 2] = a; part[blockIdx.x * 2 + 1] = b; }
}

__global__ void k_copy_neg(const double* __restrict__ src, double* __restrict__ dst, int n, double sgn) {
  const int i = blockIdx.x * blockDim.x + threadIdx.x;
  if (i < n) dst[i] = sgn * src[i];
}
__global__ void k_add_vec(const double* __restrict__ a, const double* __restrict__ b, double* __restrict__ dst, int n) {
  const int i = blockIdx.x * blockDim.x + threadIdx.x;
  if (i < n) dst[i] = a[i] + b[i];
}
__global__ __launch_bounds__(256) void k_sum_partials(const double* __restrict__ part, int nblk, int cnt,
                                                      double* __restrict__ dst) {
  __shared__ double s_red[4];
  for (int q = 0; q < cnt; ++q) {
    double t = 0.0;
    for (int i = threadIdx.x; i < nblk; i += 256) t += part[(size_t)i * cnt + q];
    double tt = block_sum256(t, s_red);
    if (threadIdx.x == 0) dst[q] = tt;
  }
}
__global__ __launch_bounds__(1024) void k_dot(int n, const double* __restrict__ a, const double* __restrict__ b, double* __restrict__ out) {
  __shared__ double s_red[17];
  double t = 0.0;
  for (int i = threadIdx.x; i < n; i += 1024) t += a[i] * b[i];
  t = block_sum1024(t, s_red);
  if (threadIdx.x == 0) *out = t;
}
void ba_copy_neg(sfm_ctx* h, const double* src, double* dst, int n, double sgn) { hipLaunchKernelGGL(k_copy_neg, dim3(cdiv(n, 256)), dim3(256), 0, h->stream, src, dst, n, sgn); }
void ba_add_vec(sfm_ctx* h, const double* a, const double* b, double* dst, int n) { hipLaunchKernelGGL(k_add_vec, dim3(cdiv(n, 256)), dim3(256), 0, h->stream, a, b, dst, n); }
void ba_dot(sfm_ctx* h, int n, const double* a, const double* b, double* out) { hipLaunchKernelGGL(k_dot, dim3(1), dim3(1024), 0, h->stream, n, a, b, out); }
void ba_sum_partials(sfm_ctx* h, const double* part, int nblk, int cnt, double* dst) { hipLaunchKernelGGL(k_sum_partials, dim3(1), dim3(256), 0, h->stream, part, nblk, cnt, dst); }

int check_problem(sfm_ctx* h, sfm_ba_problem p, Lay* L) {
  if (!h) return SFM_ERR_ARG;
  if (!p) return sfm_fail(h, SFM_ERR_ARG, "sfm_ba", "null problem");
  if (!p->workspace) return sfm_fail(h, SFM_ERR_WORKSPACE, "sfm_ba", "no workspace bound (sfm_ba_bind_workspace)");
  *L = p->L;
  return SFM_OK;
}

extern "C" int sfm_ba_set_sharded(sfm_handle h, sfm_ba_problem p, int sharded) {
  if (!h) return SFM_ERR_ARG;
  if (!p) return sfm_fail(h, SFM_ERR_ARG, "sfm_ba_set_sharded", "null problem");
  p->sharded = sharded ? 1 : 0;
  return SFM_OK;
}

void launch_build_G(sfm_ctx* h, sfm_ba_problem p, const Lay& L, double alpha, double* cg_scal) {
  double* ws = (double*)p->workspace; const int64_t N = p->n_obs, P = p->n_pts;
  DISPATCH_DT(p->cam_dim, p->precision,
    hipLaunchKernelGGL((k_build_G<DD, TT, double, GG>), dim3(cdiv(N, 256) + cdiv(P, 256)), dim3(256), 0, h->stream, N, p->pt_idx, WST(L, recA),
                       WST(L, recB), WS(L, Linv), WS(L, G), WS(L, e), WS(L, eobs), WS(L, Cp), WS(L, gp), alpha, (int)P, (unsigned)cdiv(N, 256),
                       cg_scal));
}
void launch_obs_Gtp(sfm_ctx* h, sfm_ba_problem p, const Lay& L, const double* vc) {
  double* ws = (double*)p->workspace; const int64_t N = p->n_obs;
  DISPATCH_D(p->cam_dim, hipLaunchKernelGGL((k_obs_Gtp<DD, double, GG>), dim3(cdiv(N, GTP_OBS)), dim3(256), 0, h->stream, N, p->cam_idx, WS(L, G), vc, WS(L, tmp3)));
}
void launch_backsub_points(sfm_ctx* h, sfm_ba_problem p, const Lay& L) {
  double* ws = (double*)p->workspace;
  hipLaunchKernelGGL(k_backsub, dim3((unsigned)L.nblk_pt), dim3(256), 0, h->stream, p->n_pts, p->pt_ptr, WS(L, tmp3),
                     WS(L, Linv), WS(L, e), WS(L, pp), WS(L, v), WS(L, part_pt));
}
void launch_cam_reduce_chunks(sfm_ctx* h, sfm_ba_problem p, const Lay& L, const double* vec) {
  double* ws = (double*)p->workspace;
  if (p->n_cchunks > 0)
    DISPATCH_D(p->cam_dim, hipLaunchKernelGGL((k_cam_reduce_chunks<DD, double, GG>), dim3((unsigned)p->n_cchunks), dim3(256), 0, h->stream, p->cch_beg,
                                              p->cch_end, p->cam_obs, p->cam_pt, WS(L, G), vec, WS(L, cch_part)));
}
void launch_cam_reduce_final(sfm_ctx* h, sfm_ba_problem p, const Lay& L, const double* base, double* out, bool point_sums) {
  double* ws = (double*)p->workspace; const int C = p->n_cams, s = point_sums ? 1 : 0;
  DISPATCH_D(p->cam_dim, hipLaunchKernelGGL(k_cam_reduce_final<DD>, dim3(cdiv(C, 4) + s), dim3(256), 0, h->stream, C, p->cch_ptr, WS(L, cch_part),
                                            base, out, s ? WS(L, part_pt) : (const double*)nullptr, s ? (int)L.nblk_pt : 0, s ? 2 : 0,
                                            s ? WS(L, red_q) + C * p->cam_dim : (double*)nullptr));
}

static void launch_schur_assemble(sfm_ctx* h, sfm_ba_problem p, const Lay& L, double alpha, double* einv_out, double* m_out) {
  double* ws = (double*)p->workspace;
  const int C = p->n_cams, D = p->cam_dim, n = C * D;
  const AsmShape shape = schur_assemble_shape(C);
#define ASM_LAUNCH(NB, ROUNDS)                                                                                                  \
  hipLaunchKernelGGL((k_schur_assemble<DD, NB, ROUNDS>), dim3(C, cdiv(C, NB)), dim3(128), 0, h->stream, C, p->item_ptr,          \
                     WS(L, sch_part), WS(L, B), WS(L, red_S), WS(L, cg_scal), p->cch_ptr, WS(L, cch_part), WS(L, gc),             \
                     WS(L, red_S) + (size_t)n * n, alpha, einv_out, m_out)
  DISPATCH_D(D, {
    if (shape.rounds) ASM_LAUNCH(8, true);
    else if (shape.nb == 8) ASM_LAUNCH(8, false);
    else ASM_LAUNCH(2, false);
  });
#undef ASM_LAUNCH
}
static void launch_schur_assemble_scaled(sfm_ctx* h, sfm_ba_problem p, const Lay& L, double alpha, double* St) {
  double* ws = (double*)p->workspace;
  const int C = p->n_cams, D = p->cam_dim, n = C * D;
#define ASM_LAUNCH(NB)                                                                                                          \
  hipLaunchKernelGGL((k_schur_assemble_scaled<DD, NB>), dim3(C, cdiv(C, NB)), dim3(128), 0, h->stream, C, p->item_ptr,           \
                     WS(L, sch_part), WS(L, B), St, p->cch_ptr, WS(L, cch_part), WS(L, gc), WS(L, red_S) + (size_t)n * n,         \
                     WS(L, cg_r), alpha, WS(L, cg_Minv))
  DISPATCH_D(D, {
    hipLaunchKernelGGL(k_schur_diag<DD>, dim3(C), dim3(128), 0, h->stream, C, p->item_ptr, WS(L, sch_part), WS(L, B), alpha,
                       WS(L, cg_Minv), WS(L, cg_M), WS(L, cg_scal));
    if (schur_assemble_scaled_nb(C) == 4) ASM_LAUNCH(4);
    else ASM_LAUNCH(2);
  });
#undef ASM_LAUNCH
}

extern "C" int sfm_ba_schur_build(sfm_handle h, sfm_ba_problem p, double alpha) {
  Lay L; int rc = check_problem(h, p, &L); if (rc) return rc;
  if (!(alpha > 0.0)) return sfm_fail(h, SFM_ERR_ARG, "sfm_ba_schur_build", "alpha must be > 0");
  double* ws = (double*)p->workspace;
  const int C = p->n_cams, D = p->cam_dim, n = C * D;
  const BaSwitches sw = ba_switches_from_env();
  const CamPlan plan = cam_plan(n, p->camera_solver, h->cgs_persist_off != 0, sw);
  sfm_prof_begin(h, SFM_PROF_BUILD_G);
  launch_build_G(h, p, L, alpha, WS(L, cg_scal));
  sfm_prof_end(h, SFM_PROF_BUILD_G);
  sfm_prof_begin(h, SFM_PROF_SCHUR);
  DISPATCH_DT(D, p->precision, {
    if (p->n_items > 0) {
      sfm_prof_begin(h, SFM_PROF_SCHUR_ITEMS);
      hipLaunchKernelGGL((k_schur_items<DD, double, GG>), dim3(8 * cdiv(p->xcd_max_items, SFM_SCHUR_WG_WAVES)),
                         dim3(64 * SFM_SCHUR_WG_WAVES), 0, h->stream,
                         p->xcd_ptr, p->xcd_items, p->it_first, p->it_stride, p->it_cnt, p->pair_k, p->pair_k2, WS(L, G), WS(L, sch_part),
                         p->cam_idx, p->item_ptr, p->cch_ptr, C, WS(L, eobs), WS(L, cch_part), p->has_dup ? 0 : 1);
      sfm_prof_end(h, SFM_PROF_SCHUR_ITEMS);
    }
  });
  if (p->has_dup) launch_cam_reduce_chunks(h, p, L, WS(L, e));
  const BuildFusion fuse = build_fusion(plan, p->sharded != 0, p->camera_solver, n, sw);
  p->st_alpha = -1.0;
  p->s_valid = fuse.scale ? 0 : 1;
  if (fuse.scale) {
    DenseWs dw; dense_ws_carve(WS(L, dense), n, &dw);
    launch_schur_assemble_scaled(h, p, L, alpha, dw.Lm);
    p->st_alpha = alpha;
  } else
    launch_schur_assemble(h, p, L, alpha, fuse.einv ? WS(L, cg_Minv) : (double*)nullptr, WS(L, cg_M));
  p->cg_scal_clean = 1;
  p->einv_alpha = fuse.einv ? alpha : -1.0;
  sfm_prof_end(h, SFM_PROF_SCHUR);
  SFM_LAUNCH_CHECK(h, "sfm_ba_schur_build");
  return SFM_OK;
}

int schur_materialise_S(sfm_ctx* h, sfm_ba_problem p, const Lay& L) {
  if (p->s_valid) return SFM_OK;
  launch_schur_assemble(h, p, L, 0.0, nullptr, nullptr);
  p->s_valid = 1;
  SFM_LAUNCH_CHECK(h, "schur_materialise_S");
  return SFM_OK;
}

__global__ __launch_bounds__(256) void k_pack_lower(const double* __restrict__ S, int n, double* __restrict__ Sp, int unpack_dir) {
  const int r = blockIdx.x;
  const int len = r < n ? r + 1 : n;
  const size_t off = (size_t)r * (r + 1) / 2;
  double* full = const_cast<double*>(S) + (size_t)r * n;
  for (int c = threadIdx.x; c < len; c += 256) {
    if (unpack_dir) full[c] = Sp[off + c];
    else Sp[off + c] = full[c];
  }
}

static int pack_S(sfm_handle h, sfm_ba_problem p, int unpack_dir, const char* what) {
  Lay L; int rc = check_problem(h, p, &L); if (rc) return rc;
  double* ws = (double*)p->workspace;
  const int n = p->n_cams * p->cam_dim;
  DenseWs dw; dense_ws_carve(WS(L, dense), n, &dw);
  if ((rc = schur_materialise_S(h, p, L))) return rc;
  p->st_alpha = -1.0;
  hipLaunchKernelGGL(k_pack_lower, dim3(n + 1), dim3(256), 0, h->stream, WS(L, red_S), n, dw.Lm, unpack_dir);
  SFM_LAUNCH_CHECK(h, what);
  return SFM_OK;
}
extern "C" int sfm_ba_pack_system(sfm_handle h, sfm_ba_problem p) { return pack_S(h, p, 0, "sfm_ba_pack_system"); }
extern "C" int sfm_ba_unpack_system(sfm_handle h, sfm_ba_problem p) { return pack_S(h, p, 1, "sfm_ba_unpack_system"); }

void launch_backsub(sfm_ctx* h, sfm_ba_problem p, const Lay& L, int want_q) {
  double* ws = (double*)p->workspace;
  sfm_prof_begin(h, SFM_PROF_BACKSUB);
  launch_obs_Gtp(h, p, L, WS(L, pc));
  launch_backsub_points(h, p, L);
  if (want_q) launch_cam_reduce_chunks(h, p, L, WS(L, v));
  if (want_q) launch_cam_reduce_final(h, p, L, nullptr, WS(L, red_q), true);
  else ba_sum_partials(h, WS(L, part_pt), (int)L.nblk_pt, 2, WS(L, red_q) + p->n_cams * p->cam_dim);
  sfm_prof_end(h, SFM_PROF_BACKSUB);
}

bool ba_wait_for_word(sfm_ctx* h, const volatile double* word, double want) {
  constexpr unsigned SPIN_QUERY = 4096;
  bool seen = false;
  for (unsigned spins = 1; ; ++spins) {
    if (*word == want) { seen = true; break; }
    if ((spins % SPIN_QUERY) == 0 && hipStreamQuery(h->stream) != hipErrorNotReady) break;
#if defined(__x86_64__)
    __builtin_ia32_pause();
#endif
  }
  std::atomic_thread_fence(std::memory_order_acquire);
  return seen;
}

extern "C" int sfm_ba_read_scalars(sfm_handle h, sfm_ba_problem p, double* out_host) {
  Lay L; int rc = check_problem(h, p, &L); if (rc) return rc;
  static const bool poll_on = !(getenv("SFM_POLL_SCALARS") && getenv("SFM_POLL_SCALARS")[0] == '0');
  const bool seen = poll_on && p->look_pending && ba_wait_for_word(h, p->host_sc + SFM_HSC_SEQ, p->look_seq);
  p->look_pending = 0;
  if (!seen) SFM_HIP(h, hipStreamSynchronize(h->stream));
  if (p->cg2_pending && (rc = cgs_second_system_verdict(h, p, L))) return rc;
  memcpy(out_host, p->host_sc, SFM_SC_COUNT * sizeof(double));
  return SFM_OK;
}
```

sfm_amd/csrc/ba_internal.h:

```cpp
#pragma once
#include "dense.h"
#include "ba_plan.h"

struct Lay {
  int64_t recA, recB, campre, campre2, B, gc, Cp, gp, Linv, e, v, tmp3, G, eobs, red_lin, gmax, red_S, red_q,
      red_step, pc, pp, y, tvec, scalars, part_obs, part_pt, part_x, cost_reg, regrec, dense, sch_part, cch_part, cbl_part,
      cg_r, cg_z, cg_p, cg_Ap, cg_M, cg_Minv, cg_scal, cg_mail, total;
  int64_t nblk_obs, nblk_pt;
};
constexpr int CG_SCAL_WORDS = 16;

struct sfm_ba_prob {
  sfm_ctx* h;
  int32_t n_cams, n_pts, cam_dim, apply_reg, precision;
  int64_t n_obs;
  double fx0, fy0, cx0, cy0, width, height, reg_weight;
  int32_t *cam_idx, *pt_idx;
  double* uv;
  int32_t *pt_ptr, *cam_ptr, *cam_obs, *blk_ptr, *pair_k, *pair_k2;
  int32_t* cam_pt;

  int64_t n_pairs;
  int32_t *item_ptr, *item_beg, *item_end;
  int32_t *it_first, *it_stride, *it_cnt;
  int64_t n_items;
  int32_t *xcd_ptr, *xcd_items;
  int64_t xcd_max_items;
  int32_t *cch_ptr, *cch_beg, *cch_end;
  int64_t n_cchunks;
  void* workspace;
  int64_t workspace_bytes;
  int owns_workspace;
  Lay L;
  int camera_solver, cg_state, cg_iters, cg_fallbacks;
  int cg2_pending;
  double* host_sc;
  double look_seq;
  int look_pending;
  int sharded;
  int cg_scal_clean;
  double einv_alpha;
  double st_alpha;
  int s_valid;
  int has_dup;
  int64_t pcg_fallbacks;
  double pcg_worst_relres;
  double cg_alpha;
  CgPredictor cgp;
  int cg_its_sys1;
};

constexpr int SFM_HSC_CG2 = SFM_SC_COUNT, SFM_HSC_SEQ = SFM_SC_COUNT + 8, SFM_HSC_WORDS = SFM_SC_COUNT + 16;

static inline double next_ticket(sfm_ba_prob* p) { p->look_seq += 1.0; p->look_pending = 1; return p->look_seq; }

Lay ba_layout(int64_t C, int64_t P, int64_t N, int64_t D, int64_t n_items, int64_t n_cchunks, int precision);

void* sfm_scratch(sfm_ctx* h, size_t bytes);

int ba_xnorm_partial(sfm_ctx* h, sfm_ba_problem p, const double* x);
int ba_xnorm_finish(sfm_ctx* h, sfm_ba_problem p, const double* x);
#include "ba_stages.h"
```

sfm_amd/csrc/ba_stages.h:

```cpp
#pragma once
enum { CGS_RR0 = 0, CGS_RR = 1, CGS_ITER = 2, CGS_FAIL = 3, CGS_DONE = 4,
       CGS_RR_SLOT = 5 };
enum { CGB_PAIR = 5 };
enum { CG_RZ = 0, CG_RR = 1, CG_RR0 = 2, CG_ITER = 3, CG_FAIL = 4, CG_DOT = 5 };
#pragma GCC visibility push(hidden)
int check_problem(sfm_ctx* h, sfm_ba_problem p, Lay* L);
bool ba_wait_for_word(sfm_ctx* h, const volatile double* word, double want);
void ba_copy_neg(sfm_ctx* h, const double* src, double* dst, int n, double sgn);
void ba_add_vec(sfm_ctx* h, const double* a, const double* b, double* dst, int n);
void ba_dot(sfm_ctx* h, int n, const double* a, const double* b, double* out);
void ba_sum_partials(sfm_ctx* h, const double* part, int nblk, int cnt, double* dst);
void launch_build_G(sfm_ctx* h, sfm_ba_problem p, const Lay& L, double alpha, double* cg_scal);
void launch_obs_Gtp(sfm_ctx* h, sfm_ba_problem p, const Lay& L, const double* vc);
void launch_backsub_points(sfm_ctx* h, sfm_ba_problem p, const Lay& L);
void launch_cam_reduce_chunks(sfm_ctx* h, sfm_ba_problem p, const Lay& L, const double* vec);
void launch_cam_reduce_final(sfm_ctx* h, sfm_ba_problem p, const Lay& L, const double* base, double* out, bool point_sums);
void launch_backsub(sfm_ctx* h, sfm_ba_problem p, const Lay& L, int want_q);
int schur_materialise_S(sfm_ctx* h, sfm_ba_problem p, const Lay& L);
void launch_finish_solve_pcg(sfm_ctx* h, sfm_ba_problem p, const Lay& L, int want_q, const double* dotp, const double* failp);
int cgs_second_system_verdict(sfm_ctx* h, sfm_ba_problem p, const Lay& L);
#pragma GCC visibility pop
```

sfm_amd/csrc/trf.hip:

```cpp
#include <cmath>
#include <vector>
#include "ba_internal.h"
#include "trf_loop.h"

struct sfm_trf_state_s {
  sfm_ctx* h;
  sfm_ba_problem p;
  double* x;
  double* x_new;
  sfm_trf_options opt;
  sfm_reduce_fn reduce;
  void* reduce_user;
  sfm_ba_layout lay;
  trf_core::State st;
  int n_solves;
  long long cg_iters;
};

namespace {

struct Backend {
  sfm_trf_state_s* s;
  double sc[SFM_SC_COUNT];

  int red(int64_t off_bytes, int64_t count, int op) {
    if (!s->reduce) return SFM_OK;
    int rc = s->reduce(s->reduce_user, (char*)s->p->workspace + off_bytes, count, op);
    return rc ? sfm_fail(s->h, SFM_ERR_HIP, "sfm_ba_trf", "the reduce hook failed") : SFM_OK;
  }
  int scalars() { return sfm_ba_read_scalars(s->h, s->p, sc); }

  int linearize(double* cost, double* g_norm, double* g_inf, double* hdiag) {
    int rc;
    if ((rc = sfm_ba_linearize(s->h, s->p, s->x))) return rc;
    if ((rc = red(s->lay.reduce_lin_off, s->lay.reduce_lin_count, 0))) return rc;
    if ((rc = red(s->lay.gmax_off, 2, 1))) return rc;
    if ((rc = sfm_ba_finish_linearize(s->h, s->p))) return rc;
    if ((rc = scalars())) return rc;
    *cost = sc[SFM_SC_COST]; *g_norm = std::sqrt(sc[SFM_SC_GNORM2]); *g_inf = sc[SFM_SC_GINF]; *hdiag = sc[SFM_SC_HDIAG];
    if (!std::isfinite(*cost)) return sfm_fail(s->h, SFM_ERR_NUMERIC, "sfm_ba_trf", "residuals are not finite");
    return SFM_OK;
  }
  int solve(double alpha, int want_q, double* p_norm, double* pq) {
    int rc;
    if (s->opt.solver == SFM_SOLVER_PCG) {
      const int n = s->p->n_cams * s->p->cam_dim;
      const double rtol = s->opt.pcg_rtol > 0 ? s->opt.pcg_rtol : 1e-13;
      const int mit = s->opt.pcg_max_iter > 0 ? s->opt.pcg_max_iter : 400;
      int32_t its = 0;
      if ((rc = sfm_ba_solve_pcg(s->h, s->p, alpha, want_q, rtol, mit, s->reduce, s->reduce_user, &its))) return rc;
      s->cg_iters += its;
      return after_solve(p_norm, pq);
    }
    if ((rc = sfm_ba_schur_build(s->h, s->p, alpha))) return rc;
    if (s->reduce) {
      if ((rc = sfm_ba_pack_system(s->h, s->p))) return rc;
      if ((rc = red(s->lay.reduce_Sp_off, s->lay.reduce_Sp_count, 0))) return rc;
      if ((rc = sfm_ba_unpack_system(s->h, s->p))) return rc;
    }
    if ((rc = sfm_ba_schur_solve(s->h, s->p, alpha, want_q))) return rc;
    if ((rc = red(s->lay.reduce_q_off, s->lay.reduce_q_count, 0))) return rc;
    if ((rc = sfm_ba_finish_solve(s->h, s->p, want_q))) return rc;
    return after_solve(p_norm, pq);
  }
  int after_solve(double* p_norm, double* pq) {
    int rc;
    if ((rc = scalars())) return rc;
    s->n_solves++;
    if (sc[SFM_SC_CHOL_FAIL] != 0.0)
      return sfm_fail(s->h, SFM_ERR_NUMERIC, "sfm_ba_trf",
                      sc[SFM_SC_CHOL_FAIL] == 1.0 ? "reduced camera system not positive definite"
                      : sc[SFM_SC_CHOL_FAIL] == 2.0 ? "triangular solve stalled" : "damped step is not finite");
    *p_norm = std::sqrt(sc[SFM_SC_PNORM2]); *pq = sc[SFM_SC_PQ];
    return SFM_OK;
  }
  int step(double scale, double* js2, double* gts, double* cost_new, double* step_norm, double* xnew_norm) {
    int rc;
    if ((rc = sfm_ba_step(s->h, s->p, s->x, scale, s->x_new))) return rc;
    if ((rc = red(s->lay.reduce_step_off, s->lay.reduce_step_count, 0))) return rc;
    if ((rc = sfm_ba_finish_step(s->h, s->p, s->x, scale, s->x_new))) return rc;
    if ((rc = scalars())) return rc;
    *js2 = sc[SFM_SC_JS2]; *gts = sc[SFM_SC_GTS]; *cost_new = sc[SFM_SC_COST_NEW];
    *step_norm = std::sqrt(sc[SFM_SC_SNORM2]); *xnew_norm = std::sqrt(sc[SFM_SC_XNEW_NORM2]);
    return SFM_OK;
  }
  int x_norm(double* out) {
    int rc;
    if ((rc = ba_xnorm_partial(s->h, s->p, s->x))) return rc;
    if ((rc = red(s->lay.reduce_step_off + 4 * 8, 1, 0))) return rc;
    if ((rc = ba_xnorm_finish(s->h, s->p, s->x))) return rc;
    if ((rc = scalars())) return rc;
    *out = std::sqrt(sc[SFM_SC_XNEW_NORM2]);
    return SFM_OK;
  }
  int accept() {
    const size_t bytes = ((size_t)s->p->n_cams * s->p->cam_dim + 3 * (size_t)s->p->n_pts) * sizeof(double);
    if (hipMemcpyAsync(s->x, s->x_new, bytes, hipMemcpyDeviceToDevice, s->h->stream) != hipSuccess)
      return sfm_fail(s->h, SFM_ERR_HIP, "sfm_ba_trf", "copy of the accepted iterate failed");
    return SFM_OK;
  }
};

}

extern "C" int sfm_ba_trf_begin(sfm_handle h, sfm_ba_problem p, double* x, const sfm_trf_options* opt,
                                sfm_reduce_fn reduce, void* reduce_user, sfm_trf_state* out) {
  if (!h) return SFM_ERR_ARG;
  if (!p || !x || !opt || !out) return sfm_fail(h, SFM_ERR_ARG, "sfm_ba_trf_begin", "null argument");
  if (!p->workspace) return sfm_fail(h, SFM_ERR_WORKSPACE, "sfm_ba_trf_begin", "no workspace bound (sfm_ba_bind_workspace)");
  sfm_trf_state_s* s = new sfm_trf_state_s();
  s->h = h; s->p = p; s->x = x; s->x_new = nullptr; s->opt = *opt; s->reduce = reduce; s->reduce_user = reduce_user;
  s->cg_iters = 0;
  if (reduce) p->sharded = 1;
  sfm_ba_get_layout(p, &s->lay);
  const size_t bytes = ((size_t)p->n_cams * p->cam_dim + 3 * (size_t)p->n_pts) * sizeof(double);
  if (hipMalloc((void**)&s->x_new, bytes) != hipSuccess) { delete s; return sfm_fail(h, SFM_ERR_HIP, "sfm_ba_trf_begin", "hipMalloc"); }
  Backend be{s};
  s->n_solves = 0;
  const int rc = trf_core::begin(be, s->st);
  if (rc) { (void)hipFree(s->x_new); delete s; return rc; }
  *out = s;
  return SFM_OK;
}

extern "C" int sfm_ba_trf_outer(sfm_trf_state s, int* more) {
  if (!s || !more) return SFM_ERR_ARG;
  const sfm_trf_options& o = s->opt;
  const trf_core::Options co = {o.ftol, o.xtol, o.gtol, o.max_nfev, o.max_outer, o.check_tolerances};
  Backend be{s};
  return trf_core::outer(be, s->st, co, more);
}

extern "C" int sfm_ba_trf_result(sfm_trf_state s, sfm_trf_result* out) {
  if (!s || !out) return SFM_ERR_ARG;
  out->cost = s->st.cost; out->optimality = s->st.g_inf;
  out->nfev = s->st.nfev; out->njev = s->st.njev; out->status = s->st.status < 0 ? 0 : s->st.status;
  out->n_solves = s->n_solves; out->n_outer = s->st.iteration; out->cg_iters = (int32_t)(s->cg_iters > 0x7fffffff ? 0x7fffffff : s->cg_iters);
  return SFM_OK;
}

extern "C" int sfm_ba_trf_trace(sfm_trf_state s, double* out_host, int32_t capacity_trials) {
  if (!s) return 0;
  const std::vector<double>& trace = s->st.trace;
  const int n = (int)(trace.size() / 4);
  if (out_host)
    for (int i = 0; i < n && i < capacity_trials; ++i)
      for (int q = 0; q < 4; ++q) out_host[4 * i + q] = trace[4 * (size_t)i + q];
  return n;
}

extern "C" void sfm_ba_trf_end(sfm_trf_state s) {
  if (!s) return;
  (void)hipStreamSynchronize(s->h->stream);
  if (s->x_new) (void)hipFree(s->x_new);
  delete s;
}

extern "C" int sfm_ba_run_trf(sfm_handle h, sfm_ba_problem p, double* x, const sfm_trf_options* opt,
                              sfm_reduce_fn reduce, void* reduce_user, sfm_trf_result* out) {
  if (!h) return SFM_ERR_ARG;
  if (!out) return sfm_fail(h, SFM_ERR_ARG, "sfm_ba_run_trf", "null result");
  sfm_trf_state st = nullptr;
  int rc = sfm_ba_trf_begin(h, p, x, opt, reduce, reduce_user, &st);
  if (rc) return rc;
  int more = 1;
  while (more && !(rc = sfm_ba_trf_outer(st, &more))) {}
  sfm_ba_trf_result(st, out);
  sfm_ba_trf_end(st);
  return rc;
}
```

sfm_amd/csrc/trf_loop.h:

```cpp
#pragma once
#include <cmath>
#include <vector>

namespace trf_core {

constexpr double ALPHA_FLOOR_REL = 1e-13;
constexpr int TR_COLLAPSED = 1 << 30;

struct Options { double ftol, xtol, gtol; int max_nfev, max_outer, check_tolerances; };

struct State {
  double cost = 0, g_norm = 0, g_inf = 0, hdiag = 0, x_norm = 0, Delta = 0, alpha = 0;
  int nfev = 0, njev = 0, status = -1 , iteration = 0;
  std::vector<double> trace;
};

inline void update_tr_radius(double& Delta, double actual, double predicted, double step_norm, bool bound_hit, double* ratio) {
  double r;
  if (predicted > 0) r = actual / predicted;
  else if (predicted == 0 && actual == 0) r = 1;
  else r = 0;
  if (r < 0.25) Delta = 0.25 * step_norm;
  else if (r > 0.75 && bound_hit) Delta *= 2.0;
  *ratio = r;
}

inline int check_termination(double dF, double F, double dx_norm, double x_norm, double ratio, double ftol, double xtol) {
  const bool f_ok = dF < ftol * F && ratio > 0.25;
  const bool x_ok = dx_norm < xtol * (xtol + x_norm);
  if (f_ok && x_ok) return 4;
  if (f_ok) return 2;
  if (x_ok) return 3;
  return 0;
}

template <class BE>
int solve_tr_more(BE& be, double g_norm, double Delta, double& alpha, double alpha_floor, double* p_norm_out) {
  double alpha_upper = g_norm / Delta, alpha_lower = 0.0;
  if (alpha == 0) alpha = std::fmax(0.001 * alpha_upper, std::sqrt(alpha_lower * alpha_upper));
  int rc;
  for (int it = 0; it < 10; ++it) {
    if (alpha < alpha_lower || alpha > alpha_upper) alpha = std::fmax(0.001 * alpha_upper, std::sqrt(alpha_lower * alpha_upper));
    const bool on_floor = alpha <= alpha_floor;
    if (on_floor) alpha = alpha_floor;
    if (!(alpha > 0)) return TR_COLLAPSED;
    double p_norm, pq;
    if ((rc = be.solve(alpha, 1, &p_norm, &pq))) return rc;
    const double phi = p_norm - Delta;
    if (on_floor && phi < 0) { *p_norm_out = p_norm; return 0; }
    const double phi_prime = -pq / p_norm;
    if (phi < 0) alpha_upper = alpha;
    const double ratio = phi / phi_prime;
    alpha_lower = std::fmax(alpha_lower, alpha - ratio);
    alpha -= (phi + Delta) * ratio / Delta;
    if (std::fabs(phi) < 0.01 * Delta) break;
  }
  alpha = std::fmax(std::fmax(alpha, alpha_floor), 1e-300);
  double pq;
  return be.solve(alpha, 0, p_norm_out, &pq);
}

template <class BE>
int begin(BE& be, State& s) {
  int rc = be.linearize(&s.cost, &s.g_norm, &s.g_inf, &s.hdiag);
  if (!rc) rc = be.x_norm(&s.x_norm);
  if (rc) return rc;
  s.nfev = 1; s.njev = 1;
  s.Delta = s.x_norm > 0 ? s.x_norm : 1.0;
  s.alpha = 0.0;
  s.status = -1;
  s.iteration = 0;
  return 0;
}

template <class BE>
int outer(BE& be, State& s, const Options& o, int* more) {
  *more = 0;
  if (o.max_outer >= 0 && s.iteration >= o.max_outer) return 0;
  if (s.g_inf < o.gtol && o.check_tolerances) s.status = 1;
  if (s.status >= 0 || s.nfev == o.max_nfev) return 0;
  double actual = -1.0, cost_new = s.cost, xnew_norm = s.x_norm;
  int rc;
  while (actual <= 0 && s.nfev < o.max_nfev) {
    double p_norm;
    rc = solve_tr_more(be, s.g_norm, s.Delta, s.alpha, ALPHA_FLOOR_REL * s.hdiag, &p_norm);
    if (rc == TR_COLLAPSED) { s.status = 3; return 0; }
    if (rc) return rc;
    double js2, gts, step_norm;
    if ((rc = be.step(s.Delta / p_norm, &js2, &gts, &cost_new, &step_norm, &xnew_norm))) return rc;
    const double predicted = -(0.5 * js2 + gts);
    s.nfev++;
    if (!std::isfinite(cost_new)) { s.Delta = 0.25 * step_norm; continue; }
    actual = s.cost - cost_new;
    double Delta_new = s.Delta, ratio;
    update_tr_radius(Delta_new, actual, predicted, step_norm, step_norm > 0.95 * s.Delta, &ratio);
    s.trace.push_back(s.alpha); s.trace.push_back(s.Delta); s.trace.push_back(step_norm); s.trace.push_back(actual > 0 ? 1.0 : 0.0);
    if (o.check_tolerances) {
      const int t = check_termination(actual, s.cost, step_norm, s.x_norm, ratio, o.ftol, o.xtol);
      if (t) { s.status = t; break; }
    }
    s.alpha *= s.Delta / Delta_new;
    s.Delta = Delta_new;
  }
  if (actual > 0) {
    if ((rc = be.accept())) return rc;
    s.x_norm = xnew_norm;
    s.cost = cost_new;
    double c_unused;
    if ((rc = be.linearize(&c_unused, &s.g_norm, &s.g_inf, &s.hdiag))) return rc;
    s.njev++;
  }
  s.iteration++;
  *more = 1;
  return 0;
}

}
```

Before: 253.6 LM-iterations/s.

## Speculatively enqueue Schur build with device-evaluated deferred alpha

```diff
diff --git a/include/sfm_amd.h b/include/sfm_amd.h
--- a/include/sfm_amd.h
+++ b/include/sfm_amd.h
@@ -221,6 +221,9 @@
 int  sfm_ba_trf_outer(sfm_trf_state st, int* more);
 int  sfm_ba_trf_result(sfm_trf_state st, sfm_trf_result* out);
 int  sfm_ba_trf_trace(sfm_trf_state st, double* out_host, int32_t capacity_trials);
+int  sfm_ba_trf_ahead_stats(sfm_trf_state st, int32_t* out4);
+int  sfm_debug_deferred_eval(sfm_handle h, const double* rows_dev, int32_t n, double* out_dev);
+int  sfm_debug_deferred_eval_host(const double* rows, int32_t n, double* out);
 void sfm_ba_trf_end(sfm_trf_state st);
 int  sfm_ba_run_trf(sfm_handle h, sfm_ba_problem p, double* x, const sfm_trf_options* opt,
                     sfm_reduce_fn reduce, void* reduce_user, sfm_trf_result* out);
diff --git a/sfm_amd/_lib.py b/sfm_amd/_lib.py
--- a/sfm_amd/_lib.py
+++ b/sfm_amd/_lib.py
@@ -108,6 +108,9 @@
     "sfm_ba_trf_outer": (C.c_int, [vp, C.POINTER(C.c_int)]),
     "sfm_ba_trf_result": (C.c_int, [vp, C.POINTER(TRFResultC)]),
     "sfm_ba_trf_trace": (C.c_int, [vp, vp, i32]),
+    "sfm_ba_trf_ahead_stats": (C.c_int, [vp, vp]),
+    "sfm_debug_deferred_eval": (C.c_int, [vp, vp, i32, vp]),
+    "sfm_debug_deferred_eval_host": (C.c_int, [vp, i32, vp]),
     "sfm_ba_trf_end": (None, [vp]),
     "sfm_ba_run_trf": (C.c_int, [vp, vp, vp, C.POINTER(TRFOptions), REDUCE_FN, vp, C.POINTER(TRFResultC)]),
     "sfm_ba_cost": (C.c_int, [vp, vp, vp]),
diff --git a/sfm_amd/csrc/ba.hip b/sfm_amd/csrc/ba.hip
--- a/sfm_amd/csrc/ba.hip
+++ b/sfm_amd/csrc/ba.hip
@@ -97,9 +97,16 @@
                                                  const T* __restrict__ recA, const T* __restrict__ recB,
                                                  double* __restrict__ Linv, TG* __restrict__ G,
                                                  double* __restrict__ e, double* __restrict__ eobs,
-                                                 const double* __restrict__ Cp, const double* __restrict__ gp, double alpha, int P,
+                                                 const double* __restrict__ Cp, const double* __restrict__ gp, trf_core::Deferred qa, int P,
                                                  unsigned nblk_obs, double* __restrict__ cg_scal ) {
   static_assert(GS % 2 == 0 && GS >= 3 * D, "G blocks are written as 16-byte pieces");
+  const trf_core::DeferredIn qin = trf_core::deferred_load(qa);
+  double alpha;
+  if (blockIdx.x == 0 || blockIdx.x >= nblk_obs) {
+    const bool have_alpha = trf_core::deferred_eval(qa, qin, &alpha);
+    if (blockIdx.x == 0 && threadIdx.x == 0) trf_core::deferred_echo(qa, have_alpha, alpha);
+    if (!have_alpha) return;
+  }
   if (cg_scal && blockIdx.x == 0 && threadIdx.x < CG_SCAL_WORDS) cg_scal[threadIdx.x] = 0.0;
   if (blockIdx.x >= nblk_obs) {
     const int j = (int)(blockIdx.x - nblk_obs) * 256 + (int)threadIdx.x;
@@ -150,6 +157,7 @@
 #pragma unroll
     for (int v = 0; v < VE; ++v) { const int i = (tid + 256 * j) * VE + v; s_jp[(i >> 3) * LDB + (i & 7)] = (double)lb[j][v]; }
   __syncthreads();
+  if (blockIdx.x != 0 && !trf_core::deferred_eval(qa, qin, &alpha)) return;
   double mq[6], eq[3];
   point_factor_vals(cpj, gpj, alpha, mq, eq);
   const double m00 = mq[0], m10 = mq[1], m11 = mq[2], m20 = mq[3], m21 = mq[4], m22 = mq[5];
@@ -251,7 +259,7 @@
                                                      const int* __restrict__ cam_idx,
                                                      const int* __restrict__ item_ptr, const int* __restrict__ cch_ptr, int n_cams,
                                                      const double* __restrict__ eobs, double* __restrict__ cch_part,
-                                                     int fuse_rhs) {
+                                                     int fuse_rhs, trf_core::Deferred qa ) {
   typedef int chunk_t __attribute__((ext_vector_type(4)));
   constexpr int BB = GS * (int)sizeof(T);
   static_assert(BB % 16 == 0, "a G block must be a whole number of 16-byte chunks");
@@ -265,6 +273,7 @@
   __shared__ __attribute__((aligned(16))) char s_stage[WGW][2][BPL * BB + 16];
   __shared__ double s_e[WGW][64][3];
   const int lane = threadIdx.x & 63, w = threadIdx.x >> 6;
+  const trf_core::DeferredIn qin = trf_core::deferred_load(qa);
   const int grp = blockIdx.x & 7;
   const int pos = xcd_ptr[grp] + (blockIdx.x >> 3) * WGW + w;
   if (pos >= xcd_ptr[grp + 1]) return;
@@ -272,6 +281,7 @@
   const int it = __builtin_amdgcn_readfirstlane(xcd_items[pos]);
   const int first = __builtin_amdgcn_readfirstlane(it_first[it]), stride = __builtin_amdgcn_readfirstlane(it_stride[it]);
   const int n = __builtin_amdgcn_readfirstlane(it_cnt[it]);
+  if (qa.kind != trf_core::DEF_VALUE) { double unused; if (!trf_core::deferred_eval(qa, qin, &unused)) return; }
   const int row = lane & 15, m = lane >> 4;
   const int lb = lane / CH, lc = lane - lb * CH;
   const bool loader = lb < BPL;
@@ -461,19 +471,22 @@
                                                         const double* __restrict__ B, double* __restrict__ S, double* __restrict__ cg_scal,
                                                         const int* __restrict__ cch_ptr, const double* __restrict__ cch_part,
                                                         const double* __restrict__ gc, double* __restrict__ rhs_out,
-                                                        double alpha, double* __restrict__ Einv , double* __restrict__ Efac) {
+                                                        trf_core::Deferred qa, double* __restrict__ Einv , double* __restrict__ Efac) {
+  const trf_core::DeferredIn qin = trf_core::deferred_load(qa);
   if (blockIdx.y == 0 && threadIdx.x < 64) {
     const int cc = blockIdx.x, lane = threadIdx.x, sl = lane >> 4, a = lane & 15;
     double t = 0.0;
     for (int ch = cch_ptr[cc] + sl; ch < cch_ptr[cc + 1]; ch += 4) t += cch_part[(size_t)ch * 16 + a];
     const double t1 = __shfl(t, a + 16, 64), t2 = __shfl(t, a + 32, 64), t3 = __shfl(t, a + 48, 64);
-    if (sl == 0 && a < D) rhs_out[cc * D + a] = gc[cc * D + a] - ((t + t1) + (t2 + t3));
+    double unused;
+    if (sl == 0 && a < D && trf_core::deferred_eval(qa, qin, &unused)) rhs_out[cc * D + a] = gc[cc * D + a] - ((t + t1) + (t2 + t3));
   }
   __shared__ double sOut[D][ASM_NB * D + 1];
   const int r = blockIdx.x, c_0 = blockIdx.y * ASM_NB;
   if (c_0 > r) return;
   const int nv = (r - c_0 + 1) < ASM_NB ? (r - c_0 + 1) : ASM_NB;
   const int e = threadIdx.x;
+  double alpha;
   if (e < D * D) {
     const int rr = e / D, col = e - rr * D;
     if (ROUNDS) {
@@ -499,6 +512,7 @@
     }
   }
   __syncthreads();
+  if (!trf_core::deferred_eval(qa, qin, &alpha)) return;
   if (Einv && r < c_0 + ASM_NB && e < D)
     diag_block_factor_lanes<D>(&sOut[0][(r - c_0) * D], ASM_NB * D + 1, alpha, e, r, Einv, Efac, cg_scal);
   const int n = C * D, W = nv * D;
@@ -513,8 +527,10 @@
 
 template <int D>
 __global__ __launch_bounds__(128) void k_schur_diag(int C, const int* __restrict__ item_ptr, const double* __restrict__ part,
-                                                    const double* __restrict__ B, double alpha, double* __restrict__ Einv,
+                                                    const double* __restrict__ B, trf_core::Deferred qa, double* __restrict__ Einv,
                                                     double* __restrict__ Efac, double* __restrict__ cg_scal) {
+  double alpha;
+  if (!trf_core::deferred_eval(qa, &alpha)) return;
   __shared__ double sBlk[D][D + 1];
   const int r = blockIdx.x, e = threadIdx.x;
   if (e < D * D) {
@@ -535,7 +551,9 @@
                                                                const double* __restrict__ B, double* __restrict__ St,
                                                                const int* __restrict__ cch_ptr, const double* __restrict__ cch_part,
                                                                const double* __restrict__ gc, double* __restrict__ rhs_out,
-                                                               double* __restrict__ rhs_t, double alpha, const double* __restrict__ Einv) {
+                                                               double* __restrict__ rhs_t, trf_core::Deferred qa, const double* __restrict__ Einv) {
+  double alpha;
+  if (!trf_core::deferred_eval(qa, &alpha)) return;
   constexpr int SCALED_BAND = 128 / D + 2;
   if (blockIdx.y == 0 && threadIdx.x < 64) {
     const int cc = blockIdx.x, lane = threadIdx.x, sl = lane >> 4, a = lane & 15;
@@ -816,6 +834,9 @@
 }
 
 void launch_build_G(sfm_ctx* h, sfm_ba_problem p, const Lay& L, double alpha, double* cg_scal) {
+  launch_build_G_deferred(h, p, L, trf_core::deferred_const(alpha), cg_scal);
+}
+void launch_build_G_deferred(sfm_ctx* h, sfm_ba_problem p, const Lay& L, const trf_core::Deferred& alpha, double* cg_scal) {
   double* ws = (double*)p->workspace; const int64_t N = p->n_obs, P = p->n_pts;
   DISPATCH_DT(p->cam_dim, p->precision,
     hipLaunchKernelGGL((k_build_G<DD, TT, double, GG>), dim3(cdiv(N, 256) + cdiv(P, 256)), dim3(256), 0, h->stream, N, p->pt_idx, WST(L, recA),
@@ -844,7 +865,7 @@
                                             s ? WS(L, red_q) + C * p->cam_dim : (double*)nullptr));
 }
 
-static void launch_schur_assemble(sfm_ctx* h, sfm_ba_problem p, const Lay& L, double alpha, double* einv_out, double* m_out) {
+static void launch_schur_assemble(sfm_ctx* h, sfm_ba_problem p, const Lay& L, const trf_core::Deferred& alpha, double* einv_out, double* m_out) {
   double* ws = (double*)p->workspace;
   const int C = p->n_cams, D = p->cam_dim, n = C * D;
   const AsmShape shape = schur_assemble_shape(C);
@@ -859,7 +880,7 @@
   });
 #undef ASM_LAUNCH
 }
-static void launch_schur_assemble_scaled(sfm_ctx* h, sfm_ba_problem p, const Lay& L, double alpha, double* St) {
+static void launch_schur_assemble_scaled(sfm_ctx* h, sfm_ba_problem p, const Lay& L, const trf_core::Deferred& alpha, double* St) {
   double* ws = (double*)p->workspace;
   const int C = p->n_cams, D = p->cam_dim, n = C * D;
 #define ASM_LAUNCH(NB)                                                                                                          \
@@ -875,15 +896,13 @@
 #undef ASM_LAUNCH
 }
 
-extern "C" int sfm_ba_schur_build(sfm_handle h, sfm_ba_problem p, double alpha) {
-  Lay L; int rc = check_problem(h, p, &L); if (rc) return rc;
-  if (!(alpha > 0.0)) return sfm_fail(h, SFM_ERR_ARG, "sfm_ba_schur_build", "alpha must be > 0");
+static int schur_build_launches(sfm_ctx* h, sfm_ba_problem p, const Lay& L, const trf_core::Deferred& alpha, BuildFusion* fuse_out) {
   double* ws = (double*)p->workspace;
   const int C = p->n_cams, D = p->cam_dim, n = C * D;
   const BaSwitches sw = ba_switches_from_env();
   const CamPlan plan = cam_plan(n, p->camera_solver, h->cgs_persist_off != 0, sw);
   sfm_prof_begin(h, SFM_PROF_BUILD_G);
-  launch_build_G(h, p, L, alpha, WS(L, cg_scal));
+  launch_build_G_deferred(h, p, L, alpha, WS(L, cg_scal));
   sfm_prof_end(h, SFM_PROF_BUILD_G);
   sfm_prof_begin(h, SFM_PROF_SCHUR);
   DISPATCH_DT(D, p->precision, {
@@ -892,30 +911,62 @@
       hipLaunchKernelGGL((k_schur_items<DD, double, GG>), dim3(8 * cdiv(p->xcd_max_items, SFM_SCHUR_WG_WAVES)),
                          dim3(64 * SFM_SCHUR_WG_WAVES), 0, h->stream,
                          p->xcd_ptr, p->xcd_items, p->it_first, p->it_stride, p->it_cnt, p->pair_k, p->pair_k2, WS(L, G), WS(L, sch_part),
-                         p->cam_idx, p->item_ptr, p->cch_ptr, C, WS(L, eobs), WS(L, cch_part), p->has_dup ? 0 : 1);
+                         p->cam_idx, p->item_ptr, p->cch_ptr, C, WS(L, eobs), WS(L, cch_part), p->has_dup ? 0 : 1, alpha);
       sfm_prof_end(h, SFM_PROF_SCHUR_ITEMS);
     }
   });
   if (p->has_dup) launch_cam_reduce_chunks(h, p, L, WS(L, e));
   const BuildFusion fuse = build_fusion(plan, p->sharded != 0, p->camera_solver, n, sw);
-  p->st_alpha = -1.0;
-  p->s_valid = fuse.scale ? 0 : 1;
   if (fuse.scale) {
     DenseWs dw; dense_ws_carve(WS(L, dense), n, &dw);
     launch_schur_assemble_scaled(h, p, L, alpha, dw.Lm);
-    p->st_alpha = alpha;
   } else
     launch_schur_assemble(h, p, L, alpha, fuse.einv ? WS(L, cg_Minv) : (double*)nullptr, WS(L, cg_M));
+  sfm_prof_end(h, SFM_PROF_SCHUR);
+  *fuse_out = fuse;
+  SFM_LAUNCH_CHECK(h, "sfm_ba_schur_build");
+  return SFM_OK;
+}
+static void schur_build_commit(sfm_ba_problem p, const BuildFusion& fuse, double alpha) {
+  p->st_alpha = fuse.scale ? alpha : -1.0;
+  p->s_valid = fuse.scale ? 0 : 1;
   p->cg_scal_clean = 1;
   p->einv_alpha = fuse.einv ? alpha : -1.0;
-  sfm_prof_end(h, SFM_PROF_SCHUR);
-  SFM_LAUNCH_CHECK(h, "sfm_ba_schur_build");
+}
+
+extern "C" int sfm_ba_schur_build(sfm_handle h, sfm_ba_problem p, double alpha) {
+  Lay L; int rc = check_problem(h, p, &L); if (rc) return rc;
+  if (!(alpha > 0.0)) return sfm_fail(h, SFM_ERR_ARG, "sfm_ba_schur_build", "alpha must be > 0");
+  BuildFusion fuse;
+  if ((rc = schur_build_launches(h, p, L, trf_core::deferred_const(alpha), &fuse))) return rc;
+  schur_build_commit(p, fuse, alpha);
   return SFM_OK;
+}
+
+int ba_schur_build_ahead(sfm_ctx* h, sfm_ba_problem p, trf_core::Deferred q) {
+  Lay L; int rc = check_problem(h, p, &L); if (rc) return rc;
+  double* ws = (double*)p->workspace;
+  p->echo_seq += 1.0;
+  q.sc = WS(L, scalars); q.echo = p->host_sc + SFM_HSC_ECHO; q.seq = p->echo_seq;
+  BuildFusion fuse;
+  if ((rc = schur_build_launches(h, p, L, q, &fuse))) return rc;
+  p->ahead_fuse_scale = fuse.scale ? 1 : 0; p->ahead_fuse_einv = fuse.einv ? 1 : 0;
+  return SFM_OK;
+}
+int ba_schur_build_settle(sfm_ctx* h, sfm_ba_problem p, double* alpha_out) {
+  const volatile double* e = p->host_sc + SFM_HSC_ECHO;
+  if (!ba_wait_for_word(h, e + 2, p->echo_seq)) return -1;
+  *alpha_out = e[0];
+  return e[1] != 0.0 ? 1 : 0;
+}
+void ba_schur_build_commit(sfm_ba_problem p, double alpha) {
+  BuildFusion fuse; fuse.scale = p->ahead_fuse_scale != 0; fuse.einv = p->ahead_fuse_einv != 0;
+  schur_build_commit(p, fuse, alpha);
 }
 
 int schur_materialise_S(sfm_ctx* h, sfm_ba_problem p, const Lay& L) {
   if (p->s_valid) return SFM_OK;
-  launch_schur_assemble(h, p, L, 0.0, nullptr, nullptr);
+  launch_schur_assemble(h, p, L, trf_core::deferred_const(0.0), nullptr, nullptr);
   p->s_valid = 1;
   SFM_LAUNCH_CHECK(h, "schur_materialise_S");
   return SFM_OK;
@@ -977,6 +1028,10 @@
   const bool seen = poll_on && p->look_pending && ba_wait_for_word(h, p->host_sc + SFM_HSC_SEQ, p->look_seq);
   p->look_pending = 0;
   if (!seen) SFM_HIP(h, hipStreamSynchronize(h->stream));
+  if (p->cg2_pending && p->ahead_look) {
+    const double* st = p->host_sc + SFM_HSC_CG2;
+    if (!(st[CGS_DONE] != -1.0 && st[CGS_FAIL] == 0.0 && st[CGS_DONE] != 0.0)) { p->ahead_nonnominal = 1; p->cg2_pending = 0; }
+  }
   if (p->cg2_pending && (rc = cgs_second_system_verdict(h, p, L))) return rc;
   memcpy(out_host, p->host_sc, SFM_SC_COUNT * sizeof(double));
   return SFM_OK;
diff --git a/sfm_amd/csrc/ba_internal.h b/sfm_amd/csrc/ba_internal.h
--- a/sfm_amd/csrc/ba_internal.h
+++ b/sfm_amd/csrc/ba_internal.h
@@ -1,6 +1,7 @@
 #pragma once
 #include "dense.h"
 #include "ba_plan.h"
+#include "trf_defer.h"
 
 struct Lay {
   int64_t recA, recB, campre, campre2, B, gc, Cp, gp, Linv, e, v, tmp3, G, eobs, red_lin, gmax, red_S, red_q,
@@ -48,9 +49,14 @@
   double cg_alpha;
   CgPredictor cgp;
   int cg_its_sys1;
+  double echo_seq;
+  int ahead_fuse_scale, ahead_fuse_einv;
+  int ahead_look, ahead_nonnominal;
 };
 
-constexpr int SFM_HSC_CG2 = SFM_SC_COUNT, SFM_HSC_SEQ = SFM_SC_COUNT + 8, SFM_HSC_WORDS = SFM_SC_COUNT + 16;
+constexpr int SFM_HSC_CG2 = SFM_SC_COUNT, SFM_HSC_SEQ = SFM_SC_COUNT + 8, SFM_HSC_ECHO = SFM_SC_COUNT + 9, SFM_HSC_WORDS = SFM_SC_COUNT + 16;
+static_assert(trf_core::DEF_SC_GNORM2 == SFM_SC_GNORM2 && trf_core::DEF_SC_PNORM2 == SFM_SC_PNORM2 && trf_core::DEF_SC_PQ == SFM_SC_PQ &&
+              trf_core::DEF_SC_HDIAG == SFM_SC_HDIAG, "trf_defer.h reads the scalars by these indices");
 
 static inline double next_ticket(sfm_ba_prob* p) { p->look_seq += 1.0; p->look_pending = 1; return p->look_seq; }
 
diff --git a/sfm_amd/csrc/ba_stages.h b/sfm_amd/csrc/ba_stages.h
--- a/sfm_amd/csrc/ba_stages.h
+++ b/sfm_amd/csrc/ba_stages.h
@@ -11,6 +11,10 @@
 void ba_dot(sfm_ctx* h, int n, const double* a, const double* b, double* out);
 void ba_sum_partials(sfm_ctx* h, const double* part, int nblk, int cnt, double* dst);
 void launch_build_G(sfm_ctx* h, sfm_ba_problem p, const Lay& L, double alpha, double* cg_scal);
+void launch_build_G_deferred(sfm_ctx* h, sfm_ba_problem p, const Lay& L, const trf_core::Deferred& alpha, double* cg_scal);
+int ba_schur_build_ahead(sfm_ctx* h, sfm_ba_problem p, trf_core::Deferred q);
+int ba_schur_build_settle(sfm_ctx* h, sfm_ba_problem p, double* alpha_out);
+void ba_schur_build_commit(sfm_ba_problem p, double alpha);
 void launch_obs_Gtp(sfm_ctx* h, sfm_ba_problem p, const Lay& L, const double* vc);
 void launch_backsub_points(sfm_ctx* h, sfm_ba_problem p, const Lay& L);
 void launch_cam_reduce_chunks(sfm_ctx* h, sfm_ba_problem p, const Lay& L, const double* vec);
diff --git a/sfm_amd/csrc/trf.hip b/sfm_amd/csrc/trf.hip
--- a/sfm_amd/csrc/trf.hip
+++ b/sfm_amd/csrc/trf.hip
@@ -1,4 +1,6 @@
 #include <cmath>
+#include <cstdlib>
+#include <cstring>
 #include <vector>
 #include "ba_internal.h"
 #include "trf_loop.h"
@@ -15,6 +17,11 @@
   trf_core::State st;
   int n_solves;
   long long cg_iters;
+  int ahead;
+  int pending;
+  int told_first;
+  double fa_alpha, fa_Delta;
+  int n_ahead, n_misspec, n_redo, n_void;
 };
 
 namespace {
@@ -30,12 +37,43 @@
   }
   int scalars() { return sfm_ba_read_scalars(s->h, s->p, sc); }
 
+  trf_core::MoreState more_m;
+  bool have_more = false, ahead_off = false;
+  bool ahead_ok() const { return s->ahead && !ahead_off && !s->reduce && s->opt.solver == SFM_SOLVER_DENSE && !s->p->has_dup; }
+  void ahead_more(const trf_core::MoreState& m) { more_m = m; have_more = true; }
+  void ahead_first(double alpha, double Delta) { s->told_first = 1; s->fa_alpha = alpha; s->fa_Delta = Delta; }
+  int drain() {
+    if (hipStreamSynchronize(s->h->stream) != hipSuccess) return sfm_fail(s->h, SFM_ERR_HIP, "sfm_ba_trf", "stream synchronisation failed");
+    return SFM_OK;
+  }
+  int settle(double want_alpha, bool* built) {
+    *built = false;
+    if (!s->pending) return SFM_OK;
+    s->pending = 0;
+    double used = 0.0;
+    const int r = ba_schur_build_settle(s->h, s->p, &used);
+    if (want_alpha > 0 ? (r == 1 && std::memcmp(&used, &want_alpha, sizeof(double)) == 0) : r == 0) {
+      if (want_alpha > 0) { ba_schur_build_commit(s->p, want_alpha); *built = true; }
+      else s->n_void++;
+      return SFM_OK;
+    }
+    s->n_misspec++;
+    s->ahead = 0;
+    return drain();
+  }
+
   int linearize(double* cost, double* g_norm, double* g_inf, double* hdiag) {
     int rc;
     if ((rc = sfm_ba_linearize(s->h, s->p, s->x))) return rc;
     if ((rc = red(s->lay.reduce_lin_off, s->lay.reduce_lin_count, 0))) return rc;
     if ((rc = red(s->lay.gmax_off, 2, 1))) return rc;
     if ((rc = sfm_ba_finish_linearize(s->h, s->p))) return rc;
+    if (s->told_first && ahead_ok()) {
+      trf_core::Deferred q = {trf_core::DEF_FIRST_ALPHA, s->fa_alpha, s->fa_Delta, 0, 0, 0, 0, nullptr, nullptr, 0.0};
+      if ((rc = ba_schur_build_ahead(s->h, s->p, q))) return rc;
+      s->pending = 1; s->n_ahead++;
+    }
+    s->told_first = 0;
     if ((rc = scalars())) return rc;
     *cost = sc[SFM_SC_COST]; *g_norm = std::sqrt(sc[SFM_SC_GNORM2]); *g_inf = sc[SFM_SC_GINF]; *hdiag = sc[SFM_SC_HDIAG];
     if (!std::isfinite(*cost)) return sfm_fail(s->h, SFM_ERR_NUMERIC, "sfm_ba_trf", "residuals are not finite");
@@ -52,20 +90,48 @@
       s->cg_iters += its;
       return after_solve(p_norm, pq);
     }
-    if ((rc = sfm_ba_schur_build(s->h, s->p, alpha))) return rc;
-    if (s->reduce) {
-      if ((rc = sfm_ba_pack_system(s->h, s->p))) return rc;
-      if ((rc = red(s->lay.reduce_Sp_off, s->lay.reduce_Sp_count, 0))) return rc;
-      if ((rc = sfm_ba_unpack_system(s->h, s->p))) return rc;
-    }
-    if ((rc = sfm_ba_schur_solve(s->h, s->p, alpha, want_q))) return rc;
-    if ((rc = red(s->lay.reduce_q_off, s->lay.reduce_q_count, 0))) return rc;
-    if ((rc = sfm_ba_finish_solve(s->h, s->p, want_q))) return rc;
+    bool built = false;
+    if ((rc = settle(alpha, &built))) return rc;
+    sfm_ba_prob* const p = s->p;
+    const int k_iters = p->cg_iters, k_fallbacks = p->cg_fallbacks, k_sys1 = p->cg_its_sys1;
+    const CgPredictor k_cgp = p->cgp;
+    for (int attempt = 0; ; ++attempt) {
+      if (!built && (rc = sfm_ba_schur_build(s->h, s->p, alpha))) return rc;
+      built = false;
+      if (s->reduce) {
+        if ((rc = sfm_ba_pack_system(s->h, s->p))) return rc;
+        if ((rc = red(s->lay.reduce_Sp_off, s->lay.reduce_Sp_count, 0))) return rc;
+        if ((rc = sfm_ba_unpack_system(s->h, s->p))) return rc;
+      }
+      if ((rc = sfm_ba_schur_solve(s->h, s->p, alpha, want_q))) return rc;
+      if ((rc = red(s->lay.reduce_q_off, s->lay.reduce_q_count, 0))) return rc;
+      if ((rc = sfm_ba_finish_solve(s->h, s->p, want_q))) return rc;
+      if (!(have_more && want_q && attempt == 0 && ahead_ok())) break;
+      trf_core::Deferred q = {trf_core::DEF_MORE_NEXT, more_m.alpha, more_m.lower, more_m.upper, more_m.Delta, more_m.floor, more_m.it, nullptr, nullptr, 0.0};
+      if ((rc = ba_schur_build_ahead(s->h, s->p, q))) return rc;
+      s->n_ahead++;
+      p->ahead_look = 1;
+      rc = scalars();
+      p->ahead_look = 0;
+      if (rc) return rc;
+      const bool forced = s->ahead == 2 && (s->n_ahead % 3) == 0;
+      if (!p->ahead_nonnominal && !forced) { s->pending = 1; have_more = false; return after_look(p_norm, pq); }
+      p->ahead_nonnominal = 0;
+      if ((rc = drain())) return rc;
+      s->n_redo++;
+      ahead_off = true;
+      p->cg2_pending = 0;
+      p->cg_iters = k_iters; p->cg_fallbacks = k_fallbacks; p->cg_its_sys1 = k_sys1; p->cgp = k_cgp;
+    }
+    have_more = false;
     return after_solve(p_norm, pq);
   }
   int after_solve(double* p_norm, double* pq) {
     int rc;
     if ((rc = scalars())) return rc;
+    return after_look(p_norm, pq);
+  }
+  int after_look(double* p_norm, double* pq) {
     s->n_solves++;
     if (sc[SFM_SC_CHOL_FAIL] != 0.0)
       return sfm_fail(s->h, SFM_ERR_NUMERIC, "sfm_ba_trf",
@@ -76,6 +142,8 @@
   }
   int step(double scale, double* js2, double* gts, double* cost_new, double* step_norm, double* xnew_norm) {
     int rc;
+    bool unused;
+    if ((rc = settle(0.0, &unused))) return rc;
     if ((rc = sfm_ba_step(s->h, s->p, s->x, scale, s->x_new))) return rc;
     if ((rc = red(s->lay.reduce_step_off, s->lay.reduce_step_count, 0))) return rc;
     if ((rc = sfm_ba_finish_step(s->h, s->p, s->x, scale, s->x_new))) return rc;
@@ -101,6 +169,34 @@
   }
 };
 
+}
+
+__global__ __launch_bounds__(256) void k_deferred_eval_table(int n, const double* __restrict__ rows, double* __restrict__ out) {
+  const int i = blockIdx.x * 256 + threadIdx.x;
+  if (i >= n) return;
+  const double* r = rows + (size_t)i * 24;
+  const trf_core::Deferred q = {(int)r[0], r[1], r[2], r[3], r[4], r[5], (int)r[6], r + 8, nullptr, 0.0};
+  double v = 0.0;
+  const bool ok = trf_core::deferred_eval(q, &v);
+  out[2 * i] = ok ? 1.0 : 0.0; out[2 * i + 1] = ok ? v : 0.0;
+}
+extern "C" int sfm_debug_deferred_eval(sfm_handle h, const double* rows_dev, int32_t n, double* out_dev) {
+  if (!h) return SFM_ERR_ARG;
+  if (!rows_dev || !out_dev || n < 0) return sfm_fail(h, SFM_ERR_ARG, "sfm_debug_deferred_eval", "bad argument");
+  if (n > 0) hipLaunchKernelGGL(k_deferred_eval_table, dim3(cdiv(n, 256)), dim3(256), 0, h->stream, n, rows_dev, out_dev);
+  SFM_LAUNCH_CHECK(h, "sfm_debug_deferred_eval");
+  return SFM_OK;
+}
+extern "C" int sfm_debug_deferred_eval_host(const double* rows, int32_t n, double* out) {
+  if (!rows || !out) return SFM_ERR_ARG;
+  for (int i = 0; i < n; ++i) {
+    const double* r = rows + (size_t)i * 24; const double* sc = r + 8;
+    double v = 0.0;
+    const bool ok = trf_core::deferred_value((int)r[0], r[1], r[2], r[3], r[4], r[5], (int)r[6], sc[SFM_SC_GNORM2], sc[SFM_SC_PNORM2],
+                                             sc[SFM_SC_PQ], sc[SFM_SC_HDIAG], &v);
+    out[2 * i] = ok ? 1.0 : 0.0; out[2 * i + 1] = ok ? v : 0.0;
+  }
+  return SFM_OK;
 }
 
 extern "C" int sfm_ba_trf_begin(sfm_handle h, sfm_ba_problem p, double* x, const sfm_trf_options* opt,
@@ -111,6 +207,8 @@
   sfm_trf_state_s* s = new sfm_trf_state_s();
   s->h = h; s->p = p; s->x = x; s->x_new = nullptr; s->opt = *opt; s->reduce = reduce; s->reduce_user = reduce_user;
   s->cg_iters = 0;
+  { const char* e = getenv("SFM_TRF_AHEAD"); s->ahead = e ? atoi(e) : 1; if (s->ahead < 0 || s->ahead > 2) s->ahead = 1; }
+  s->pending = 0; s->told_first = 0; s->fa_alpha = s->fa_Delta = 0.0; s->n_ahead = s->n_misspec = s->n_redo = s->n_void = 0;
   if (reduce) p->sharded = 1;
   sfm_ba_get_layout(p, &s->lay);
   const size_t bytes = ((size_t)p->n_cams * p->cam_dim + 3 * (size_t)p->n_pts) * sizeof(double);
@@ -136,6 +234,12 @@
   out->cost = s->st.cost; out->optimality = s->st.g_inf;
   out->nfev = s->st.nfev; out->njev = s->st.njev; out->status = s->st.status < 0 ? 0 : s->st.status;
   out->n_solves = s->n_solves; out->n_outer = s->st.iteration; out->cg_iters = (int32_t)(s->cg_iters > 0x7fffffff ? 0x7fffffff : s->cg_iters);
+  return SFM_OK;
+}
+
+extern "C" int sfm_ba_trf_ahead_stats(sfm_trf_state s, int32_t* out4) {
+  if (!s || !out4) return SFM_ERR_ARG;
+  out4[0] = s->n_ahead; out4[1] = s->n_misspec; out4[2] = s->n_redo; out4[3] = s->n_void;
   return SFM_OK;
 }
 
diff --git a/sfm_amd/csrc/trf_defer.h b/sfm_amd/csrc/trf_defer.h
--- /dev/null
+++ b/sfm_amd/csrc/trf_defer.h
@@ -0,0 +1,106 @@
+#pragma once
+#include <cmath>
+
+#if defined(__HIPCC__)
+#define TRF_HD __host__ __device__ inline
+#else
+#define TRF_HD inline
+#endif
+
+namespace trf_core {
+
+constexpr double ALPHA_FLOOR_REL = 1e-13;
+
+struct MoreState { double alpha, lower, upper, Delta, floor; int it; };
+enum { MORE = 0, FINAL = 1, INTERIOR = 2 };
+
+#if defined(__clang__)
+#define TRF_NO_CONTRACT _Pragma("clang fp contract(off)")
+#else
+#define TRF_NO_CONTRACT
+#endif
+
+TRF_HD MoreState first_alpha(double carried_alpha, double Delta, double gnorm2, double hdiag) {
+  TRF_NO_CONTRACT
+  MoreState m;
+  m.upper = sqrt(gnorm2) / Delta; m.lower = 0.0; m.Delta = Delta; m.floor = ALPHA_FLOOR_REL * hdiag; m.it = 0;
+  m.alpha = carried_alpha;
+  if (m.alpha == 0) m.alpha = fmax(0.001 * m.upper, sqrt(m.lower * m.upper));
+  return m;
+}
+TRF_HD bool more_enter(MoreState& m, double* alpha_out) {
+  TRF_NO_CONTRACT
+  if (m.alpha < m.lower || m.alpha > m.upper) m.alpha = fmax(0.001 * m.upper, sqrt(m.lower * m.upper));
+  if (m.alpha <= m.floor) m.alpha = m.floor;
+  *alpha_out = m.alpha;
+  return m.alpha > 0;
+}
+TRF_HD int more_advance_norm(MoreState& m, double p_norm, double pq, double* alpha_final) {
+  TRF_NO_CONTRACT
+  const bool on_floor = m.alpha <= m.floor;
+  const double phi = p_norm - m.Delta;
+  if (on_floor && phi < 0) return INTERIOR;
+  const double phi_prime = -pq / p_norm;
+  if (phi < 0) m.upper = m.alpha;
+  const double ratio = phi / phi_prime;
+  m.lower = fmax(m.lower, m.alpha - ratio);
+  m.alpha -= (phi + m.Delta) * ratio / m.Delta;
+  m.it++;
+  if (fabs(phi) < 0.01 * m.Delta || m.it >= 10) {
+    *alpha_final = fmax(fmax(m.alpha, m.floor), 1e-300);
+    return FINAL;
+  }
+  return MORE;
+}
+TRF_HD int more_advance(MoreState& m, double pnorm2, double pq, double* alpha_final) {
+  return more_advance_norm(m, sqrt(pnorm2), pq, alpha_final);
+}
+TRF_HD double step_scale(double Delta, double pnorm2) { TRF_NO_CONTRACT return Delta / sqrt(pnorm2); }
+
+enum { DEF_VALUE = 0, DEF_MORE_NEXT = 1, DEF_FIRST_ALPHA = 2, DEF_STEP_SCALE = 3 };
+struct Deferred { int kind; double a, b, c, d, e; int it; const double* sc; double* echo; double seq; };
+constexpr int DEF_SC_GNORM2 = 1, DEF_SC_PNORM2 = 3, DEF_SC_PQ = 4, DEF_SC_HDIAG = 11;
+
+TRF_HD bool deferred_value(int kind, double a, double b, double c, double d, double e, int it,
+                           double gnorm2, double pnorm2, double pq, double hdiag, double* out) {
+  if (kind == DEF_VALUE) { *out = a; return true; }
+  if (kind == DEF_STEP_SCALE) { *out = step_scale(a, pnorm2); return true; }
+  MoreState m;
+  if (kind == DEF_FIRST_ALPHA) m = first_alpha(a, b, gnorm2, hdiag);
+  else {
+    m.alpha = a; m.lower = b; m.upper = c; m.Delta = d; m.floor = e; m.it = it;
+    const int v = more_advance(m, pnorm2, pq, out);
+    if (v == INTERIOR) return false;
+    if (v == FINAL) return true;
+  }
+  return more_enter(m, out);
+}
+
+#if defined(__HIPCC__)
+__device__ __forceinline__ bool deferred_eval(const Deferred& q, double* out) {
+  if (q.kind == DEF_VALUE) { *out = q.a; return true; }
+  const double* sc = q.sc;
+  return deferred_value(q.kind, q.a, q.b, q.c, q.d, q.e, q.it, sc[DEF_SC_GNORM2], sc[DEF_SC_PNORM2], sc[DEF_SC_PQ], sc[DEF_SC_HDIAG], out);
+}
+struct DeferredIn { double gnorm2, pnorm2, pq, hdiag; };
+__device__ __forceinline__ DeferredIn deferred_load(const Deferred& q) {
+  DeferredIn in = {0.0, 0.0, 0.0, 0.0};
+  if (q.kind != DEF_VALUE) { const double* sc = q.sc; in.gnorm2 = sc[DEF_SC_GNORM2]; in.pnorm2 = sc[DEF_SC_PNORM2]; in.pq = sc[DEF_SC_PQ]; in.hdiag = sc[DEF_SC_HDIAG]; }
+  return in;
+}
+__device__ __forceinline__ bool deferred_eval(const Deferred& q, const DeferredIn& in, double* out) {
+  if (q.kind == DEF_VALUE) { *out = q.a; return true; }
+  return deferred_value(q.kind, q.a, q.b, q.c, q.d, q.e, q.it, in.gnorm2, in.pnorm2, in.pq, in.hdiag, out);
+}
+__device__ __forceinline__ void deferred_echo(const Deferred& q, bool ok, double val) {
+  if (q.kind == DEF_VALUE || !q.echo) return;
+  ((volatile double*)q.echo)[0] = val;
+  ((volatile double*)q.echo)[1] = ok ? 1.0 : 0.0;
+  __threadfence_system();
+  ((volatile double*)q.echo)[2] = q.seq;
+}
+#endif
+
+static inline Deferred deferred_const(double v) { Deferred q = {DEF_VALUE, v, 0, 0, 0, 0, 0, nullptr, nullptr, 0.0}; return q; }
+
+}
diff --git a/sfm_amd/csrc/trf_loop.h b/sfm_amd/csrc/trf_loop.h
--- a/sfm_amd/csrc/trf_loop.h
+++ b/sfm_amd/csrc/trf_loop.h
@@ -1,10 +1,12 @@
 #pragma once
 #include <cmath>
+#include <type_traits>
+#include <utility>
 #include <vector>
+#include "trf_defer.h"
 
 namespace trf_core {
 
-constexpr double ALPHA_FLOOR_REL = 1e-13;
 constexpr int TR_COLLAPSED = 1 << 30;
 
 struct Options { double ftol, xtol, gtol; int max_nfev, max_outer, check_tolerances; };
@@ -34,28 +36,27 @@
   return 0;
 }
 
+template <class BE, class = void> struct has_ahead : std::false_type {};
+template <class BE> struct has_ahead<BE, std::void_t<decltype(std::declval<BE&>().ahead_more(std::declval<const MoreState&>()))>> : std::true_type {};
+template <class BE> inline void tell_more(BE& be, const MoreState& m) { if constexpr (has_ahead<BE>::value) be.ahead_more(m); }
+template <class BE> inline void tell_first(BE& be, double alpha, double Delta) { if constexpr (has_ahead<BE>::value) be.ahead_first(alpha, Delta); }
+
 template <class BE>
 int solve_tr_more(BE& be, double g_norm, double Delta, double& alpha, double alpha_floor, double* p_norm_out) {
-  double alpha_upper = g_norm / Delta, alpha_lower = 0.0;
-  if (alpha == 0) alpha = std::fmax(0.001 * alpha_upper, std::sqrt(alpha_lower * alpha_upper));
+  MoreState m;
+  m.upper = g_norm / Delta; m.lower = 0.0; m.Delta = Delta; m.floor = alpha_floor; m.it = 0; m.alpha = alpha;
+  if (m.alpha == 0) m.alpha = std::fmax(0.001 * m.upper, std::sqrt(m.lower * m.upper));
   int rc;
-  for (int it = 0; it < 10; ++it) {
-    if (alpha < alpha_lower || alpha > alpha_upper) alpha = std::fmax(0.001 * alpha_upper, std::sqrt(alpha_lower * alpha_upper));
-    const bool on_floor = alpha <= alpha_floor;
-    if (on_floor) alpha = alpha_floor;
-    if (!(alpha > 0)) return TR_COLLAPSED;
+  for (;;) {
+    const bool positive = more_enter(m, &alpha);
+    if (!positive) return TR_COLLAPSED;
     double p_norm, pq;
+    tell_more(be, m);
     if ((rc = be.solve(alpha, 1, &p_norm, &pq))) return rc;
-    const double phi = p_norm - Delta;
-    if (on_floor && phi < 0) { *p_norm_out = p_norm; return 0; }
-    const double phi_prime = -pq / p_norm;
-    if (phi < 0) alpha_upper = alpha;
-    const double ratio = phi / phi_prime;
-    alpha_lower = std::fmax(alpha_lower, alpha - ratio);
-    alpha -= (phi + Delta) * ratio / Delta;
-    if (std::fabs(phi) < 0.01 * Delta) break;
+    const int v = more_advance_norm(m, p_norm, pq, &alpha);
+    if (v == INTERIOR) { *p_norm_out = p_norm; return 0; }
+    if (v == FINAL) break;
   }
-  alpha = std::fmax(std::fmax(alpha, alpha_floor), 1e-300);
   double pq;
   return be.solve(alpha, 0, p_norm_out, &pq);
 }
@@ -107,6 +108,7 @@
     s.x_norm = xnew_norm;
     s.cost = cost_new;
     double c_unused;
+    if (s.status < 0 && s.nfev < o.max_nfev && !(o.max_outer >= 0 && s.iteration + 1 >= o.max_outer)) tell_first(be, s.alpha, s.Delta);
     if ((rc = be.linearize(&c_unused, &s.g_norm, &s.g_inf, &s.hdiag))) return rc;
     s.njev++;
   }
```

New measurement: 216.6 LM-iterations/s. -14.6%, worse.
